# wei-zeng98/piano-a2s

Measured on AMD Instinct MI355X. Metric: training clips/sec (12 s, 5-bar), higher is better.
Workload: dtype f32

## Files before the change

include/a2s.h:

```cpp
#ifndef A2S_H
#define A2S_H
#include <stddef.h>
#include <stdint.h>
#ifdef __cplusplus
extern "C" {
#endif

#define A2S_OK 0
#define A2S_ERR_ARG (-1)
#define A2S_ERR_HIP (-2)
#define A2S_ERR_WORKSPACE (-3)

const char* a2s_last_error(void);
int a2s_version(void);
long long a2s_launch_count(void);

int a2s_gemm_f32(void* stream, int M, int N, int K, float alpha, const float* A, long sAm, long sAk,
                 const float* B, long sBk, long sBn, float beta, float* C, long ldc, const float* bias, int act,
                 int batch, long bsA, long bsB, long bsC, int splitk, float* workspace, size_t workspace_bytes);
int a2s_gemm_f32_affine(void* stream, int M, int N, int K, float alpha, const float* A, long sAm, long sAk, const float* B, long sBk,
                        long sBn, float beta, float* C, long ldc, const float* bias, int act, int batch, long bsA, long bsB, long bsC,
                        int splitk, float* workspace, size_t workspace_bytes, const float* a_scale, const float* a_shift, int a_period,
                        const float* b_scale, const float* b_shift, int b_period);
int a2s_gemm_f32_bnstats(void* stream, int M, int N, int K, const float* A, long sAm, long sAk, const float* B, long sBk, long sBn, float* C, long ldc,
                         const float* y, const float* mean, const float* invstd, const float* scale, const float* shift, int period, float* partial);
int a2s_gemm_f32_affine_scaled(void* stream, int M, int N, int K, float alpha, const float* A, long sAm, long sAk, const float* B, long sBk,
                               long sBn, float beta, float* C, long ldc, const float* bias, int act, int batch, long bsA, long bsB, long bsC,
                               int splitk, float* workspace, size_t workspace_bytes, const float* a_scale, const float* a_shift, int a_period,
                               const float* b_scale, const float* b_shift, int b_period, const float* a_absmax, const float* b_absmax);
int a2s_gemm_f32_bnstats_scaled(void* stream, int M, int N, int K, const float* A, long sAm, long sAk, const float* B, long sBk, long sBn, float* C, long ldc,
                                const float* y, const float* mean, const float* invstd, const float* scale, const float* shift, int period, float* partial,
                                const float* a_absmax, const float* b_absmax);
int a2s_linear_dgrad_bnstats(void* stream, int M, int N, int K, const float* dz, long lda, const float* Wt, float* da, long ldc, const float* y,
                             const float* mean, const float* invstd, const float* scale, const float* shift, int period, float* partial,
                             const float* dz_absmax, const float* w_absmax, float* workspace, size_t workspace_bytes, float* da_absmax_out);
int a2s_linear_fwd(void* stream, int M, int N, int K, const float* y, long lda, const float* W, float* z, long ldc, const float* scale, const float* shift,
                   int period, const float* y_absmax, const float* w_absmax, float* workspace, size_t workspace_bytes);
int a2s_linear_fwd_eligible(int M, int N, int K, int period);
int a2s_linear_wgrad(void* stream, int M, int N, int K, const float* dz, long ldz, const float* y, long lda, float* G, long ldg, const float* scale,
                     const float* shift, int period, const float* dz_absmax, const float* y_absmax, float* workspace, size_t workspace_bytes);
size_t a2s_linear_wgrad_ws_bytes(int M, int K);
int a2s_linear_wgrad_eligible(int M, int N, int K, int period);
int a2s_tallk_wgrad(void* stream, int M, int Np, int K, const float* P, long ldp, const float* A, long lda, float* G, long ldg, int transposed, float* bias,
                    const float* p_absmax, const float* a_absmax, float* workspace, size_t workspace_bytes);
size_t a2s_tallk_wgrad_ws_bytes(int M, int Np, int K);
int a2s_tallk_wgrad_eligible(int M, int Np, int K, long ldp, long lda, long ldg, int transposed);
size_t a2s_linear_dgrad_ws_bytes(int N, int K);
int a2s_linear_dgrad_blocks(int M);
int a2s_linear_dgrad_eligible(int M, int N, int K, int period);
int a2s_absmax(void* stream, const float* x, long n, float* out);
int a2s_gemm_bnstats_blocks(int M, int period);
size_t a2s_gemm_workspace_bytes(int M, int N, int batch, int splitk);
int a2s_gemm_pick_splitk(int M, int N, int K, int batch);
void a2s_gemm_debug_tile(int cfg);
int a2s_debug_set(const char* key, int value);
int a2s_debug_get(const char* key);
int a2s_env_check(void);
int a2s_persist_abort_latch(void* device_word);

int a2s_conv3x3(void* stream, const float* x, const float* w, float* y, const float* in_scale, const float* in_shift,
                float* stat_partial, int B, int T, int F, int Cin, int Cout, int flip, float* workspace);
int a2s_conv3x3_ranged(void* stream, const float* x, const float* w, float* y, const float* in_scale, const float* in_shift, const float* in_absmax,
                       float* stat_partial, float* out_absmax, int B, int T, int F, int Cin, int Cout, float* workspace);
int a2s_conv3x3_stat_blocks(int B, int T, int F, int Cin);
int a2s_conv3x3_dgrad_bnstats(void* stream, const float* dy, const float* w, float* g, const float* yl, const float* yl_mean, const float* yl_invstd,
                              const float* yl_scale, const float* yl_shift, float* stat_partial, int B, int T, int F, int Cin, int Cout,
                              float* workspace);
int a2s_bn_bwd_from_partial(void* stream, const float* g, const float* x, const float* mean, const float* invstd, const float* scale, const float* shift,
                            float* dgamma, float* dbeta, float* dx , const float* partial, int nblocks, float* c12, long rows, int C, int F);
int a2s_conv3x3_dgrad_bnstats_scaled(void* stream, const float* dy, const float* w, float* g, const float* yl, const float* yl_mean, const float* yl_invstd,
                                     const float* yl_scale, const float* yl_shift, float* stat_partial, int B, int T, int F, int Cin, int Cout,
                                     float* workspace, const float* dy_absmax);
int a2s_conv3x3_dgrad_bnstats_ranged(void* stream, const float* dy, const float* w, float* g, const float* yl, const float* yl_mean, const float* yl_invstd,
                                     const float* yl_scale, const float* yl_shift, float* stat_partial, int B, int T, int F, int Cin, int Cout,
                                     float* workspace, const float* dy_absmax, float* g_absmax_out);
int a2s_bn_bwd_from_partial_amax(void* stream, const float* g, const float* x, const float* mean, const float* invstd, const float* scale, const float* shift,
                                 float* dgamma, float* dbeta, float* dx, const float* partial, int nblocks, float* c12, long rows, int C, int F,
                                 float* dx_absmax);
size_t a2s_conv3x3_workspace_floats(int Cin);
int a2s_bn_finalize(void* stream, const float* partial, int nblocks, int C, double count, const float* gamma,
                    const float* beta, float* running_mean, float* running_var, long long* num_batches_tracked,
                    float* mean, float* invstd, float* scale, float* shift, float eps, float momentum, int training);
int a2s_bn_relu_apply(void* stream, const float* x, float* y, const float* scale, const float* shift, long n, int C, int F);
int a2s_col_stats(void* stream, const float* x, float* partial, long rows, int C, int rows_per_block);
int a2s_bn1d_relu_dropout(void* stream, const float* x, float* y, const float* scale, const float* shift,
                          const uint8_t* keep_mask, float inv_keep, long n, int C);

int a2s_gru_gates_fwd(void* stream, const float* gi, long ldgi, const float* gh, long ldgh, const float* hprev, long ldhp,
                      float* hout, long ldho, float* hout2, long ldho2, float* save, int R, int H);
int a2s_gru_seq_fwd(void* stream, const float* gi_all, long gi_bstride, long gi_tstride, const float* w_hh,
                    const float* b_hh, float* out, long out_bstride, long out_tstride, float* hbuf, float* gh,
                    float* save, float* hn, int B, int T, int H, int reverse, float* workspace, size_t workspace_bytes);

int a2s_attn_step_fwd(void* stream, const float* keys, const float* enc, const float* q, long ldq, const float* v,
                      float* ctx, long ldctx, float* ctx2, long ldctx2, float* attw, int B, int T, int H,
                      const int* n_done, int n_rows_total, float* workspace);
int a2s_attn_step_fwd_rows(void* stream, const float* keys, const float* enc, const float* q, long ldq, const float* v, float* ctx,
                           long ldctx, float* ctx2, long ldctx2, float* attw, int R, int T, int H, float* workspace, int n_clips,
                           const int* clip_order, const int* clip_rank, const int* row_until, int n_active, int step);
size_t a2s_attn_workspace_floats(int B, int T, int H);
size_t a2s_attn_workspace_floats_fused(int n_clips, int T, int H, int groups);

int a2s_log_softmax_rows(void* stream, const float* x, long ldx, float* y, long ldy, int* argmax_out, int R, int V);
int a2s_embed_rows(void* stream, const float* table, const long long* ids64, const int* ids32, long id_stride,
                   int const_id, float* out, long ldo, int col0, int R, int E, const uint8_t* keep_mask, float inv_keep);

typedef struct a2s_note_dec_args {
    const float* attn_w; const float* attn_b; const float* attn_v;
    const float* w_ih; const float* w_hh; const float* b_ih; const float* b_hh;
    const float* out_w; const float* out_b; const float* emb;
    const float* keys; const float* enc;
    float* h; float* x; float* q; float* gates; float* attw; float* o;
    float* gh; float* gi; float* logits;
    float* probs; long probs_bstride;
    const long long* gt; long gt_bstride;
    const uint8_t* tf_flags;
    const uint8_t* drop; float inv_keep;
    int* argmax_out; long am_bstride;
    int* eos_seen; long long* lengths; int* n_done;
    int* steps_exec;
    float* attn_ws;
    float* gemm_ws; size_t gemm_ws_bytes;
    int* t_base;
    const int* clip_order;
    const int* clip_rank;
    const int* row_until;
    const int* n_active;
    int n_clips;
    const int* m_active;
    const int* row_list;
    const int* n_rows_active;
    int R, T, H, E, V, steps, poll, eos_id;
    int use_graph;
    float* step_ws; size_t step_ws_floats;
    const int* tf_flags_dev;
    float* persist_ws; size_t persist_ws_bytes;
} a2s_note_dec_args;
int a2s_note_decoder_fwd(void* stream, const a2s_note_dec_args* args, int* steps_done);
int a2s_grammar_argmax_rows(void* stream, const float* x, long ldx, float* y, long ldy, const signed char* next_state, int n_states, int* row_state,
                            int* choice_out, int R, int V);
int a2s_note_decoder_fwd_grammar(void* stream, const a2s_note_dec_args* args, const signed char* next_state, int n_states, int* row_state, int* steps_done);
int a2s_grammar_launches(void);
#define A2S_BEAM_MAX 4
typedef struct a2s_beam_args {
    int K; float alpha;
    const signed char* next_state; int n_states;
    int pad_id;
    int* row_state;
    float* score; int* finished;
    int* done_count;
    int* token_hist; int* parent_hist; float* score_hist;
    float* probs_scratch;
    int* ids_out; long long* lengths_out; float* score_out;
} a2s_beam_args;
int a2s_note_decoder_fwd_beam(void* stream, const a2s_note_dec_args* args, const a2s_beam_args* beam, int* steps_done);
int a2s_beam_step(void* stream, const a2s_beam_args* beam, const float* logits, long ldl, const float* emb, float* xnext, long ldx, float* h, int h_cols,
                  float* q, int q_cols, int* n_done, int* steps_exec, int B, int V, int E, int t, int max_steps, int eos_id);
int a2s_beam_backtrack(void* stream, const a2s_beam_args* beam, float* probs, long probs_bstride, const int* steps_exec, int B, int V, int max_steps, int eos_id);
int a2s_beam_launches(void);
typedef struct a2s_align_args {
    float* attw_step;
    int* peak; float* weight; float* centroid;
    long out_stride;
    const signed char* next_state; int n_states;
    int* row_state;
} a2s_align_args;
int a2s_attn_align_rows(void* stream, const float* attw, long ldw, int R, int T, int* peak_out, float* weight_out, float* centroid_out, long out_stride);
int a2s_note_decoder_fwd_align(void* stream, const a2s_note_dec_args* args, const a2s_align_args* align, int* steps_done);
int a2s_align_launches(void);

int a2s_render_notes(void* stream, const int* programs, int rows_per_clip, int n_samples, float* wave, long wave_bstride, int B);
int a2s_render_launches(void);
int a2s_note_decoder_fwd_pair(void* stream_upper, void* stream_lower, const a2s_note_dec_args* upper, const a2s_note_dec_args* lower,
                              const int* pair_order, const int* pair_rank, const int* pair_n_active, int* steps_done_upper, int* steps_done_lower);
size_t a2s_note_step_workspace_floats(int H, int E);
size_t a2s_note_decoder_persist_ws_bytes(int n_clips, int R, int steps);
size_t a2s_note_decoder_bwd_persist_ws_bytes(int n_clips);

int a2s_staff_emb_fwd(void* stream, const float* note_emb, const float* const* gru_w, const long long* ids64,
                      const int* ids32, long id_bstride, const long long* lengths, long len_stride, float* out,
                      long ldo, int col0, float* hsave, int R, int maxlen, int E, int S);


int a2s_log_softmax_bwd_rows(void* stream, const float* g, const float* y, long outer_stride, int inner, float* dx,
                             int R, int V, int n_outer, int time_major);
int a2s_gru_gates_bwd(void* stream, const float* dh_a, long lda, const float* dh_b, long ldb, const float* save,
                      const float* hprev, long ldhp, float* dgi, long ldgi, float* dgh, long ldgh, float* dgh2, long ldgh2,
                      float* dhprev, long lddp, int R, int H);
int a2s_attn_step_bwd(void* stream, const float* keys, const float* enc, const float* q, long ldq, const float* v,
                      const float* attw, const float* ctx, long ldctx, const float* dctx_a, long ldda, const float* dctx_b,
                      long lddb, float* dctx_out, long lddo, float* dq, long lddq, float* ds_out, int B, int T, int H, float* workspace);
int a2s_attn_step_bwd_rows(void* stream, const float* keys, const float* enc, const float* q, long ldq, const float* v, const float* attw,
                           const float* ctx, long ldctx, const float* dctx_a, long ldda, const float* dctx_b, long lddb, float* dctx_out,
                           long lddo, float* dq, long lddq, float* ds_out, int R, int T, int H, float* workspace, int n_clips,
                           const int* clip_order, const int* clip_rank, const int* row_until, int n_active, int step);
int a2s_attn_dk_accum(void* stream, const float* keys, const float* q_all, const float* ds_all, const float* v, float* dK,
                      float* dv_partial, int B, int T, int S, int H, const int* row_until, int groups);
int a2s_attn_dk_blocks(int B, int T);
int a2s_attn_denc_accum(void* stream, const float* attw_all, const float* dctx_all, float* dEnc, int B, int T, int S, int H2,
// ... 95 lines not shown
```

piano_a2s_amd/csrc/a2s_api.hip:

```cpp
#define A2S_SWITCHES_IMPL
#include "a2s_internal.h"

thread_local char a2s_err_msg[512] = {0};
long long a2s_launch_counter = 0;

#define ST ((hipStream_t)stream)

extern "C" {

const char* a2s_last_error(void) { return a2s_err_msg; }
int a2s_version(void) { return 1; }
long long a2s_launch_count(void) { return __atomic_load_n(&a2s_launch_counter, __ATOMIC_RELAXED); }

int a2s_gemm_f32(void* stream, int M, int N, int K, float alpha, const float* A, long sAm, long sAk, const float* B, long sBk,
                 long sBn, float beta, float* C, long ldc, const float* bias, int act, int batch, long bsA, long bsB, long bsC,
                 int splitk, float* workspace, size_t workspace_bytes) {
    return a2s_gemm_impl(ST, M, N, K, alpha, A, sAm, sAk, B, sBk, sBn, beta, C, ldc, bias, act, batch, bsA, bsB, bsC, splitk,
                         workspace, workspace_bytes);
}
int a2s_gemm_f32_affine(void* stream, int M, int N, int K, float alpha, const float* A, long sAm, long sAk, const float* B, long sBk,
                        long sBn, float beta, float* C, long ldc, const float* bias, int act, int batch, long bsA, long bsB, long bsC,
                        int splitk, float* workspace, size_t workspace_bytes, const float* a_scale, const float* a_shift, int a_period,
                        const float* b_scale, const float* b_shift, int b_period) {
    return a2s_gemm_affine_impl(ST, M, N, K, alpha, A, sAm, sAk, B, sBk, sBn, beta, C, ldc, bias, act, batch, bsA, bsB, bsC, splitk,
                                workspace, workspace_bytes, a_scale, a_shift, a_period, b_scale, b_shift, b_period,
                                nullptr, nullptr, nullptr, nullptr, nullptr, nullptr, 0, 0, nullptr, nullptr);
}
int a2s_gemm_f32_affine_scaled(void* stream, int M, int N, int K, float alpha, const float* A, long sAm, long sAk, const float* B, long sBk,
                               long sBn, float beta, float* C, long ldc, const float* bias, int act, int batch, long bsA, long bsB, long bsC,
                               int splitk, float* workspace, size_t workspace_bytes, const float* a_scale, const float* a_shift, int a_period,
                               const float* b_scale, const float* b_shift, int b_period, const float* a_absmax, const float* b_absmax) {
    return a2s_gemm_affine_impl(ST, M, N, K, alpha, A, sAm, sAk, B, sBk, sBn, beta, C, ldc, bias, act, batch, bsA, bsB, bsC, splitk,
                                workspace, workspace_bytes, a_scale, a_shift, a_period, b_scale, b_shift, b_period,
                                nullptr, nullptr, nullptr, nullptr, nullptr, nullptr, 0, 1, a_absmax, b_absmax);
}
int a2s_gemm_f32_bnstats_scaled(void* stream, int M, int N, int K, const float* A, long sAm, long sAk, const float* B, long sBk, long sBn, float* C, long ldc,
                                const float* y, const float* mean, const float* invstd, const float* scale, const float* shift, int period, float* partial,
                                const float* a_absmax, const float* b_absmax) {
    return a2s_gemm_affine_impl(ST, M, N, K, 1.f, A, sAm, sAk, B, sBk, sBn, 0.f, C, ldc, nullptr, 0, 1, 0, 0, 0, 1, nullptr, 0,
                                nullptr, nullptr, 0, nullptr, nullptr, 0, y, mean, invstd, scale, shift, partial, period, 1, a_absmax, b_absmax);
}
int a2s_absmax(void* stream, const float* x, long n, float* out) { return a2s_absmax_impl(ST, x, n, out); }
int a2s_linear_dgrad_bnstats(void* stream, int M, int N, int K, const float* dz, long lda, const float* Wt, float* da, long ldc, const float* y,
                             const float* mean, const float* invstd, const float* scale, const float* shift, int period, float* partial,
                             const float* dz_absmax, const float* w_absmax, float* workspace, size_t workspace_bytes, float* da_absmax_out) {
    return a2s_linear_dgrad_bnstats_impl(ST, M, N, K, dz, lda, Wt, 1, K, da, ldc, y, mean, invstd, scale, shift, period, partial, dz_absmax, w_absmax,
                                         workspace, workspace_bytes, da_absmax_out);
}
size_t a2s_linear_dgrad_ws_bytes(int N, int K) { return a2s_linear_dgrad_ws_bytes_impl(N, K); }
int a2s_linear_fwd(void* stream, int M, int N, int K, const float* y, long lda, const float* W, float* z, long ldc, const float* scale, const float* shift,
                   int period, const float* y_absmax, const float* w_absmax, float* workspace, size_t workspace_bytes) {
    return a2s_linear_fwd_impl(ST, M, N, K, y, lda, W, z, ldc, scale, shift, period, y_absmax, w_absmax, workspace, workspace_bytes);
}
int a2s_linear_wgrad(void* stream, int M, int N, int K, const float* dz, long ldz, const float* y, long lda, float* G, long ldg, const float* scale,
                     const float* shift, int period, const float* dz_absmax, const float* y_absmax, float* workspace, size_t workspace_bytes) {
    return a2s_linear_wgrad_impl(ST, M, N, K, dz, ldz, y, lda, G, ldg, scale, shift, period, dz_absmax, y_absmax, workspace, workspace_bytes);
}
size_t a2s_linear_wgrad_ws_bytes(int M, int K) { return a2s_linear_wgrad_ws_bytes_impl(M, K); }
int a2s_linear_wgrad_eligible(int M, int N, int K, int period) { return a2s_linear_wgrad_ok(M, N, K, 256, 4, 4, period, nullptr, nullptr, nullptr) ? 1 : 0; }
int a2s_tallk_wgrad(void* stream, int M, int Np, int K, const float* P, long ldp, const float* A, long lda, float* G, long ldg, int transposed, float* bias,
                    const float* p_absmax, const float* a_absmax, float* workspace, size_t workspace_bytes) {
    return a2s_tallk_wgrad_impl(ST, M, Np, K, P, ldp, A, lda, G, ldg, transposed, bias, p_absmax, a_absmax, workspace, workspace_bytes);
}
size_t a2s_tallk_wgrad_ws_bytes(int M, int Np, int K) { return a2s_tallk_wgrad_ws_bytes_impl(M, Np, K); }
int a2s_tallk_wgrad_eligible(int M, int Np, int K, long ldp, long lda, long ldg, int transposed) {
    return a2s_tallk_wgrad_ok(M, Np, K, ldp, lda, ldg, transposed, nullptr, nullptr, nullptr, nullptr) ? 1 : 0;
}
int a2s_linear_fwd_eligible(int M, int N, int K, int period) { return a2s_linear_fwd_ok(M, N, K, 4, 4, period, nullptr, nullptr, nullptr) ? 1 : 0; }
int a2s_linear_dgrad_blocks(int M) { return a2s_linear_dgrad_blocks_impl(M); }
int a2s_linear_dgrad_eligible(int M, int N, int K, int period) {
    return a2s_linear_dgrad_ok(M, N, K, 4, 1, K, 4, period, nullptr, nullptr, nullptr, nullptr) ? 1 : 0;
}
int a2s_gemm_f32_bnstats(void* stream, int M, int N, int K, const float* A, long sAm, long sAk, const float* B, long sBk, long sBn, float* C, long ldc,
                         const float* y, const float* mean, const float* invstd, const float* scale, const float* shift, int period, float* partial) {
    return a2s_gemm_affine_impl(ST, M, N, K, 1.f, A, sAm, sAk, B, sBk, sBn, 0.f, C, ldc, nullptr, 0, 1, 0, 0, 0, 1, nullptr, 0,
                                nullptr, nullptr, 0, nullptr, nullptr, 0, y, mean, invstd, scale, shift, partial, period, 0, nullptr, nullptr);
}
int a2s_gemm_bnstats_blocks(int M, int period) { return a2s_cdiv(M, 128) * a2s_gemm_bnstats_slots(period); }
size_t a2s_gemm_workspace_bytes(int M, int N, int batch, int splitk) { return a2s_gemm_workspace_bytes_impl(M, N, batch, splitk); }
int a2s_gemm_pick_splitk(int M, int N, int K, int batch) { return a2s_gemm_pick_splitk_impl(M, N, K, batch); }
void a2s_gemm_debug_tile(int cfg) { a2s_gemm_debug_tile_impl(cfg); }
size_t a2s_note_step_workspace_floats(int H, int E) { return a2s_note_step_workspace_floats_impl(H, E); }
int a2s_debug_set(const char* key, int value) {
    if (!key) return A2S_ERR_ARG;
    const int id = a2s_switch_find(key);
    if (id >= 0) { a2s_switch_store(id, value); return A2S_OK; }
    if (!strcmp(key, "attn_deferred_fast")) { a2s_attn_deferred_fast = value ? 1 : 0; return A2S_OK; }
    if (!strcmp(key, "tallk_wgrad")) { a2s_tallk_wgrad_on = value ? 1 : 0; return A2S_OK; }
    if (!strcmp(key, "tallk_wgrad_max_splits")) { a2s_tallk_wgrad_max_splits = value > 0 ? value : 0; return A2S_OK; }
    if (!strcmp(key, "gemm_tile")) { a2s_gemm_debug_tile_impl(value); return A2S_OK; }
    snprintf(a2s_err_msg, sizeof(a2s_err_msg), "a2s_debug_set: unknown key %s", key);
    return A2S_ERR_ARG;
}
int a2s_env_check(void) {
    if (const char* e = a2s_switch_env_error()) A2S_FAIL(A2S_ERR_ARG, "%s: expected a decimal number >= 0", e);
    return A2S_OK;
}

int a2s_persist_abort_latch(void* device_word) { a2s_persist_latch_set(device_word); return A2S_OK; }

int a2s_debug_get(const char* key) {
    if (!key) return -1;
    const int id = a2s_switch_find(key);
    if (id == A2S_SW_attn_pair_fused_rows) return a2s_attn_pair_fused_rows();
    if (id >= 0) return a2s_sw((a2s_switch)id);
    if (!strcmp(key, "attn_pair_launches")) return (int)a2s_attn_pair_launches();
    if (!strcmp(key, "attn_pair_bwd_launches")) return (int)a2s_attn_pair_bwd_launches();
    if (!strcmp(key, "attn_deferred_fast")) return a2s_attn_deferred_fast;
    if (!strcmp(key, "tallk_wgrad")) return a2s_tallk_wgrad_on;
    if (!strcmp(key, "tallk_wgrad_max_splits")) return a2s_tallk_wgrad_max_splits;
    if (!strcmp(key, "tallk_wgrad_launches")) return (int)a2s_tallk_wgrad_launches();
    if (!strcmp(key, "attn_dk_ahead_launches")) return (int)a2s_attn_dk_ahead_launches();
    if (!strcmp(key, "attn_denc_launches")) return (int)a2s_attn_denc_launches();
    if (!strcmp(key, "dec_mid_launches")) return a2s_dec_mid_launches();
    if (!strcmp(key, "dec_persist_launches")) return a2s_dec_persist_launches();
    if (!strcmp(key, "edit_distance_launches")) return (int)a2s_edit_distance_launches();
    if (!strcmp(key, "conv_rows16_c20_launches")) return (int)a2s_conv_rows16_c20_launches();
    if (!strcmp(key, "device_cus")) return a2s_device_geometry().cus;
    if (!strcmp(key, "device_xccs")) return a2s_device_geometry().xccs;
    return -1;
}

int a2s_conv3x3(void* stream, const float* x, const float* w, float* y, const float* in_scale, const float* in_shift,
                float* stat_partial, int B, int T, int F, int Cin, int Cout, int flip, float* workspace) {
    return a2s_conv3x3_impl(ST, x, w, y, in_scale, in_shift, stat_partial, B, T, F, Cin, Cout, flip, workspace, nullptr, nullptr, nullptr, nullptr, nullptr, nullptr,
                            nullptr, nullptr);
}
int a2s_conv3x3_ranged(void* stream, const float* x, const float* w, float* y, const float* in_scale, const float* in_shift, const float* in_absmax,
                       float* stat_partial, float* out_absmax, int B, int T, int F, int Cin, int Cout, float* workspace) {
    return a2s_conv3x3_impl(ST, x, w, y, in_scale, in_shift, stat_partial, B, T, F, Cin, Cout, 0, workspace, nullptr, nullptr, nullptr, nullptr, nullptr, nullptr,
                            in_absmax, out_absmax);
}
int a2s_conv3x3_dgrad_bnstats(void* stream, const float* dy, const float* w, float* g, const float* yl, const float* yl_mean, const float* yl_invstd,
                              const float* yl_scale, const float* yl_shift, float* stat_partial, int B, int T, int F, int Cin, int Cout,
                              float* workspace) {
    if (!yl) { snprintf(a2s_err_msg, sizeof(a2s_err_msg), "conv3x3_dgrad_bnstats: yl is required"); return A2S_ERR_ARG; }
    return a2s_conv3x3_impl(ST, dy, w, g, nullptr, nullptr, stat_partial, B, T, F, Cin, Cout, 1, workspace, yl, yl_mean, yl_invstd, yl_scale, yl_shift, nullptr, nullptr, nullptr);
}
int a2s_conv3x3_dgrad_bnstats_scaled(void* stream, const float* dy, const float* w, float* g, const float* yl, const float* yl_mean, const float* yl_invstd,
                                     const float* yl_scale, const float* yl_shift, float* stat_partial, int B, int T, int F, int Cin, int Cout,
                                     float* workspace, const float* dy_absmax) {
    if (!yl) { snprintf(a2s_err_msg, sizeof(a2s_err_msg), "conv3x3_dgrad_bnstats_scaled: yl is required"); return A2S_ERR_ARG; }
    return a2s_conv3x3_impl(ST, dy, w, g, nullptr, nullptr, stat_partial, B, T, F, Cin, Cout, 1, workspace, yl, yl_mean, yl_invstd, yl_scale, yl_shift, dy_absmax, nullptr, nullptr);
}
int a2s_conv3x3_dgrad_bnstats_ranged(void* stream, const float* dy, const float* w, float* g, const float* yl, const float* yl_mean, const float* yl_invstd,
                                     const float* yl_scale, const float* yl_shift, float* stat_partial, int B, int T, int F, int Cin, int Cout,
                                     float* workspace, const float* dy_absmax, float* g_absmax_out) {
    if (!yl) { snprintf(a2s_err_msg, sizeof(a2s_err_msg), "conv3x3_dgrad_bnstats_ranged: yl is required"); return A2S_ERR_ARG; }
    return a2s_conv3x3_impl(ST, dy, w, g, nullptr, nullptr, stat_partial, B, T, F, Cin, Cout, 1, workspace, yl, yl_mean, yl_invstd, yl_scale, yl_shift, dy_absmax, nullptr, g_absmax_out);
}
int a2s_bn_bwd_from_partial(void* stream, const float* g, const float* x, const float* mean, const float* invstd, const float* scale, const float* shift,
                            float* dgamma, float* dbeta, float* dx, const float* partial, int nblocks, float* c12, long rows, int C, int F) {
    return a2s_bn_bwd_from_partial_impl(ST, g, x, mean, invstd, scale, shift, dgamma, dbeta, dx, partial, nblocks, c12, rows, C, F, nullptr);
}
int a2s_bn_bwd_from_partial_amax(void* stream, const float* g, const float* x, const float* mean, const float* invstd, const float* scale, const float* shift,
                                 float* dgamma, float* dbeta, float* dx, const float* partial, int nblocks, float* c12, long rows, int C, int F,
                                 float* dx_absmax) {
    return a2s_bn_bwd_from_partial_impl(ST, g, x, mean, invstd, scale, shift, dgamma, dbeta, dx, partial, nblocks, c12, rows, C, F, dx_absmax);
}
size_t a2s_conv3x3_workspace_floats(int Cin) { return a2s_conv3x3_workspace_floats_impl(Cin); }
int a2s_conv3x3_stat_blocks(int B, int T, int F, int Cin) { return a2s_conv3x3_stat_blocks_impl(B, T, F, Cin); }
int a2s_bn_finalize(void* stream, const float* partial, int nblocks, int C, double count, const float* gamma, const float* beta,
                    float* running_mean, float* running_var, long long* nbt, float* mean, float* invstd, float* scale,
                    float* shift, float eps, float momentum, int training) {
    return a2s_bn_finalize_impl(ST, partial, nblocks, C, count, gamma, beta, running_mean, running_var, nbt, mean, invstd, scale,
                                shift, eps, momentum, training);
}
int a2s_bn_relu_apply(void* stream, const float* x, float* y, const float* scale, const float* shift, long n, int C, int F) {
    return a2s_bn_relu_apply_impl(ST, x, y, scale, shift, n, C, F);
}
int a2s_col_stats(void* stream, const float* x, float* partial, long rows, int C, int rows_per_block) {
    return a2s_col_stats_impl(ST, x, partial, rows, C, rows_per_block);
}
int a2s_bn1d_relu_dropout(void* stream, const float* x, float* y, const float* scale, const float* shift, const uint8_t* keep_mask,
                          float inv_keep, long n, int C) {
    return a2s_bn1d_relu_dropout_impl(ST, x, y, scale, shift, keep_mask, inv_keep, n, C);
}
int a2s_gru_gates_fwd(void* stream, const float* gi, long ldgi, const float* gh, long ldgh, const float* hprev, long ldhp,
                      float* hout, long ldho, float* hout2, long ldho2, float* save, int R, int H) {
    return a2s_gru_gates_fwd_impl(ST, gi, ldgi, gh, ldgh, hprev, ldhp, hout, ldho, hout2, ldho2, save, R, H);
}
int a2s_gru_seq_fwd(void* stream, const float* gi_all, long gi_bstride, long gi_tstride, const float* w_hh, const float* b_hh,
                    float* out, long out_bstride, long out_tstride, float* hbuf, float* gh, float* save, float* hn, int B, int T,
                    int H, int reverse, float* workspace, size_t workspace_bytes) {
    return a2s_gru_seq_fwd_impl(ST, gi_all, gi_bstride, gi_tstride, w_hh, b_hh, out, out_bstride, out_tstride, hbuf, gh, save, hn,
                                B, T, H, reverse, workspace, workspace_bytes);
}
int a2s_attn_step_fwd(void* stream, const float* keys, const float* enc, const float* q, long ldq, const float* v, float* ctx,
                      long ldctx, float* ctx2, long ldctx2, float* attw, int B, int T, int H, const int* n_done, int n_rows_total, float* workspace) {
    return a2s_attn_step_fwd_impl(ST, keys, enc, q, ldq, v, ctx, ldctx, ctx2, ldctx2, attw, B, T, H, n_done, n_rows_total, workspace, nullptr);
}
int a2s_attn_step_fwd_rows(void* stream, const float* keys, const float* enc, const float* q, long ldq, const float* v, float* ctx,
                           long ldctx, float* ctx2, long ldctx2, float* attw, int R, int T, int H, float* workspace, int n_clips,
                           const int* clip_order, const int* clip_rank, const int* row_until, int n_active, int step) {
    a2s_attn_rows rows = {clip_order, clip_rank, row_until, n_clips, n_active, step};
    return a2s_attn_step_fwd_impl(ST, keys, enc, q, ldq, v, ctx, ldctx, ctx2, ldctx2, attw, R, T, H, nullptr, 0, workspace, &rows);
}
size_t a2s_attn_workspace_floats(int B, int T, int H) { return a2s_attn_workspace_floats_impl(B, T, H, 1); }
size_t a2s_attn_workspace_floats_fused(int n_clips, int T, int H, int groups) { return a2s_attn_workspace_floats_impl(n_clips, T, H, groups); }
int a2s_log_softmax_rows(void* stream, const float* x, long ldx, float* y, long ldy, int* argmax_out, int R, int V) {
    return a2s_log_softmax_rows_impl(ST, x, ldx, y, ldy, argmax_out, R, V);
}
int a2s_embed_rows(void* stream, const float* table, const long long* ids64, const int* ids32, long id_stride, int const_id,
                   float* out, long ldo, int col0, int R, int E, const uint8_t* keep_mask, float inv_keep) {
    return a2s_embed_rows_impl(ST, table, ids64, ids32, id_stride, const_id, out, ldo, col0, R, E, keep_mask, inv_keep);
}
int a2s_note_decoder_fwd(void* stream, const a2s_note_dec_args* args, int* steps_done) {
    if (!args) { snprintf(a2s_err_msg, sizeof(a2s_err_msg), "note_decoder_fwd: null args"); return A2S_ERR_ARG; }
    return a2s_note_decoder_fwd_impl(ST, *args, steps_done);
}
int a2s_grammar_argmax_rows(void* stream, const float* x, long ldx, float* y, long ldy, const signed char* next_state, int n_states, int* row_state,
                            int* choice_out, int R, int V) {
    return a2s_grammar_argmax_rows_impl(ST, x, ldx, y, ldy, next_state, n_states, row_state, choice_out, R, V);
}
int a2s_note_decoder_fwd_grammar(void* stream, const a2s_note_dec_args* args, const signed char* next_state, int n_states, int* row_state, int* steps_done) {
    if (!args) { snprintf(a2s_err_msg, sizeof(a2s_err_msg), "note_decoder_fwd_grammar: null args"); return A2S_ERR_ARG; }
    const a2s_grammar_ref g = {next_state, n_states, row_state};
    return a2s_note_decoder_fwd_grammar_impl(ST, *args, g, steps_done);
}
int a2s_grammar_launches(void) { return a2s_grammar_launches_impl(); }
int a2s_note_decoder_fwd_beam(void* stream, const a2s_note_dec_args* args, const a2s_beam_args* beam, int* steps_done) {
    if (!args || !beam) { snprintf(a2s_err_msg, sizeof(a2s_err_msg), "note_decoder_fwd_beam: null args"); return A2S_ERR_ARG; }
    return a2s_note_decoder_fwd_beam_impl(ST, *args, *beam, steps_done);
}
int a2s_beam_step(void* stream, const a2s_beam_args* beam, const float* logits, long ldl, const float* emb, float* xnext, long ldx, float* h, int h_cols,
                  float* q, int q_cols, int* n_done, int* steps_exec, int B, int V, int E, int t, int max_steps, int eos_id) {
    if (!beam) { snprintf(a2s_err_msg, sizeof(a2s_err_msg), "beam_step: null args"); return A2S_ERR_ARG; }
    const a2s_beam_args& g = *beam;
    const BeamStepArgs a = {logits, ldl, emb, xnext, ldx, h, h_cols, q, q_cols, g.next_state, g.n_states, g.row_state, g.score, g.finished, g.done_count,
                            g.token_hist, g.parent_hist, g.score_hist, g.probs_scratch, n_done, steps_exec, B, g.K, V, E, t, max_steps, eos_id, g.pad_id};
    return a2s_beam_step_finalize_impl(ST, a);
}
int a2s_beam_backtrack(void* stream, const a2s_beam_args* beam, float* probs, long probs_bstride, const int* steps_exec, int B, int V, int max_steps, int eos_id) {
    if (!beam) { snprintf(a2s_err_msg, sizeof(a2s_err_msg), "beam_backtrack: null args"); return A2S_ERR_ARG; }
    const a2s_beam_args& g = *beam;
    const BeamBackArgs a = {g.score, g.token_hist, g.parent_hist, g.probs_scratch, probs, probs_bstride, g.ids_out, (long)max_steps, g.lengths_out, g.score_out,
                            steps_exec, g.alpha, B, g.K, V, max_steps, eos_id, g.pad_id};
    return a2s_beam_backtrack_impl(ST, a);
}
int a2s_beam_launches(void) { return a2s_beam_launches_impl(); }
int a2s_attn_align_rows(void* stream, const float* attw, long ldw, int R, int T, int* peak_out, float* weight_out, float* centroid_out, long out_stride) {
    return a2s_attn_align_rows_impl(ST, attw, ldw, R, T, peak_out, weight_out, centroid_out, out_stride);
}
int a2s_note_decoder_fwd_align(void* stream, const a2s_note_dec_args* args, const a2s_align_args* align, int* steps_done) {
    if (!args || !align) { snprintf(a2s_err_msg, sizeof(a2s_err_msg), "note_decoder_fwd_align: null args"); return A2S_ERR_ARG; }
    return a2s_note_decoder_fwd_align_impl(ST, *args, *align, steps_done);
}
int a2s_align_launches(void) { return a2s_align_launches_impl(); }
int a2s_render_notes(void* stream, const int* programs, int rows_per_clip, int n_samples, float* wave, long wave_bstride, int B) {
    return a2s_render_notes_impl(ST, programs, rows_per_clip, n_samples, wave, wave_bstride, B);
}
int a2s_render_launches(void) { return a2s_render_launches_impl(); }
int a2s_note_decoder_fwd_pair(void* stream_upper, void* stream_lower, const a2s_note_dec_args* upper, const a2s_note_dec_args* lower,
                              const int* pair_order, const int* pair_rank, const int* pair_n_active, int* steps_done_upper, int* steps_done_lower) {
    if (!upper || !lower) { snprintf(a2s_err_msg, sizeof(a2s_err_msg), "note_decoder_fwd_pair: null args"); return A2S_ERR_ARG; }
    return a2s_note_decoder_fwd_pair_impl((hipStream_t)stream_upper, (hipStream_t)stream_lower, *upper, *lower, pair_order, pair_rank, pair_n_active,
                                          steps_done_upper, steps_done_lower);
}
int a2s_staff_emb_fwd(void* stream, const float* note_emb, const float* const* gru_w, const long long* ids64, const int* ids32,
                      long id_bstride, const long long* lengths, long len_stride, float* out, long ldo, int col0, float* hsave,
                      int R, int maxlen, int E, int S) {
    if (!gru_w) { snprintf(a2s_err_msg, sizeof(a2s_err_msg), "staff_emb_fwd: null weight table"); return A2S_ERR_ARG; }
    return a2s_staff_emb_fwd_impl(ST, note_emb, gru_w, ids64, ids32, id_bstride, lengths, len_stride, out, ldo, col0, hsave, R,
                                  maxlen, E, S);
// ... 163 lines not shown
```

piano_a2s_amd/csrc/a2s_internal.h:

```cpp
#pragma once
#include "a2s_common.h"
#include "../../include/a2s.h"
#include "a2s_switches.h"

static inline int a2s_attn_pair_fused_rows(void) {
    const int cap = a2s_sw(A2S_SW_dec_fused_max_rows), v = a2s_sw(A2S_SW_attn_pair_fused_rows);
    return v < cap ? v : cap;
}
static inline unsigned a2s_persist_dbg(void) {
    return (a2s_sw(A2S_SW_persist_force_agent) ? PERSIST_DBG_FORCE_AGENT : 0u) | (a2s_sw(A2S_SW_persist_inject_abort) ? PERSIST_DBG_INJECT_ABORT : 0u);
}

int a2s_absmax_impl(hipStream_t st, const float* x, long n, float* out);
size_t a2s_gemm_workspace_bytes_impl(int M, int N, int batch, int splitk);
int a2s_gemm_pick_splitk_impl(int M, int N, int K, int batch);
int a2s_gemm_bnstats_slots(int period);
void a2s_gemm_debug_tile_impl(int cfg);
int a2s_gemm_affine_impl(hipStream_t st, int M, int N, int K, float alpha, const float* A, long sAm, long sAk,
    const float* B, long sBk, long sBn, float beta, float* C, long ldc, const float* bias, int act,
    int batch, long bsA, long bsB, long bsC, int splitk, float* ws, size_t ws_bytes,
    const float* a_scale, const float* a_shift, int a_period, const float* b_scale, const float* b_shift, int b_period,
    const float* ep_y, const float* ep_mean, const float* ep_invstd, const float* ep_scale, const float* ep_shift,
    float* ep_partial, int ep_period, int two_term, const float* a_absmax, const float* b_absmax);
int a2s_gemm_impl(hipStream_t st, int M, int N, int K, float alpha, const float* A, long sAm, long sAk,
    const float* B, long sBk, long sBn, float beta, float* C, long ldc, const float* bias, int act,
    int batch, long bsA, long bsB, long bsC, int splitk, float* ws, size_t ws_bytes);

size_t a2s_linear_dgrad_ws_bytes_impl(int N, int K);
int a2s_linear_dgrad_blocks_impl(int M);
bool a2s_linear_dgrad_ok(int M, int N, int K, long lda, long sBk, long sBn, long ldc, int period, const void* A, const void* B, const void* C, const void* y);
int a2s_linear_dgrad_bnstats_impl(hipStream_t st, int M, int N, int K, const float* A, long lda, const float* Wt, long sBk, long sBn, float* C, long ldc,
    const float* ep_y, const float* mean, const float* invstd, const float* scale, const float* shift, int period,
    float* partial, const float* a_absmax, const float* b_absmax, float* ws, size_t ws_bytes, float* c_absmax_out);
bool a2s_linear_fwd_ok(int M, int N, int K, long lda, long ldc, int period, const void* A, const void* W, const void* C);
int a2s_linear_fwd_impl(hipStream_t st, int M, int N, int K, const float* A, long lda, const float* W, float* C, long ldc, const float* a_scale,
    const float* a_shift, int period, const float* a_absmax, const float* w_absmax, float* ws, size_t ws_bytes);
size_t a2s_linear_wgrad_ws_bytes_impl(int M, int K);
bool a2s_linear_wgrad_ok(int M, int N, int K, long ldz, long lda, long ldg, int period, const void* dz, const void* A, const void* G);
int a2s_linear_wgrad_impl(hipStream_t st, int M, int N, int K, const float* dz, long ldz, const float* A, long lda, float* G, long ldg, const float* a_scale,
    const float* a_shift, int period, const float* dz_absmax, const float* a_absmax, float* ws, size_t ws_bytes);
extern int a2s_tallk_wgrad_on;
extern int a2s_tallk_wgrad_max_splits;
long a2s_tallk_wgrad_launches(void);
size_t a2s_tallk_wgrad_ws_bytes_impl(int M, int Np, int K);
bool a2s_tallk_wgrad_ok(int M, int Np, int K, long ldp, long lda, long ldg, int transposed, const void* P, const void* A, const void* G, const void* bias);
int a2s_tallk_wgrad_impl(hipStream_t st, int M, int Np, int K, const float* P, long ldp, const float* A, long lda, float* G, long ldg, int transposed,
    float* bias, const float* p_absmax, const float* a_absmax, float* ws, size_t ws_bytes);

int a2s_act_bound_impl(hipStream_t st, const float* scale, const float* shift, const float* absmax, int C, float* out);
size_t a2s_conv3x3_workspace_floats_impl(int Cin);
int a2s_conv3x3_impl(hipStream_t st, const float* x, const float* w, float* y, const float* in_scale,
    const float* in_shift, float* stat_partial, int B, int T, int F, int Cin, int Cout, int flip, float* ws,
    const float* yl, const float* yl_mean, const float* yl_invstd, const float* yl_scale, const float* yl_shift,
    const float* x_absmax, const float* in_absmax, float* out_absmax);
int a2s_conv3x3_stat_blocks_impl(int B, int T, int F, int Cin);
int a2s_bn_finalize_impl(hipStream_t st, const float* partial, int nblocks, int C, double count, const float* gamma,
    const float* beta, float* running_mean, float* running_var, long long* nbt, float* mean,
    float* invstd, float* scale, float* shift, float eps, float momentum, int training);
int a2s_bn_relu_apply_impl(hipStream_t st, const float* x, float* y, const float* scale, const float* shift, long n, int C, int F);
int a2s_col_stats_impl(hipStream_t st, const float* x, float* partial, long rows, int C, int rows_per_block);
int a2s_bn1d_relu_dropout_impl(hipStream_t st, const float* x, float* y, const float* scale, const float* shift,
    const uint8_t* mask, float inv_keep, long n, int C);
size_t a2s_conv3x3_wgrad_workspace_bytes_impl(int Cin, int Cout);
int a2s_conv3x3_wgrad_impl(hipStream_t st, const float* dy, const float* x, const float* in_scale, const float* in_shift, float* dW,
    float* ws, size_t ws_bytes, int B, int T, int F, int Cin, int Cout, const float* bn_y, const float* bn_mean,
    const float* bn_invstd, const float* bn_scale, const float* bn_shift, const float* bn_c12, float* dy_out,
    const float* dy_absmax, const float* act_absmax);
int a2s_bn_bwd_impl(hipStream_t st, const float* g, const float* x, const float* mean, const float* invstd, const float* scale,
    const float* shift, const uint8_t* mask, float inv_keep, float* dgamma, float* dbeta, float* dx, float* partial,
    float* c12, long rows, int C, int F, float* dx_absmax);
int a2s_bn_bwd_from_partial_impl(hipStream_t st, const float* g, const float* x, const float* mean, const float* invstd, const float* scale,
    const float* shift, float* dgamma, float* dbeta, float* dx, const float* partial, int nblocks, float* c12,
    long rows, int C, int F, float* dx_absmax);
int a2s_bn_bwd_stats_impl(hipStream_t st, const float* g, const float* x, const float* mean, const float* invstd, const float* scale,
    const float* shift, const uint8_t* mask, float inv_keep, float* partial, float* sums, long rows, int C, int F);
int a2s_bn_bwd_apply_impl(hipStream_t st, const float* g, const float* x, const float* mean, const float* invstd, const float* scale,
    const float* shift, const uint8_t* mask, float inv_keep, const float* sums_local, const float* sums_global,
    double count_global, float* dgamma, float* dbeta, float* dx, float* c12, long rows, int C, int F);
int a2s_bn_bwd_sums_from_partial_impl(hipStream_t st, const float* partial, int nblocks, int C, float* sums);
int a2s_bn_bwd_c12_from_sums_impl(hipStream_t st, const float* sums_local, const float* sums_global, double count_global, float* dgamma, float* dbeta,
    float* c12, int C);
size_t a2s_bn_bwd_partial_floats_impl(long rows, int C, int F);

int a2s_channel_absmax_impl(hipStream_t st, const float* x, long rows, int C, int F, float* out);
bool a2s_conv_rows_eligible(int F, int Cin);
int a2s_conv_rows_blocks(int B, int T, int F);
size_t a2s_conv_rows_workspace_floats(int Cin);
long a2s_conv_rows16_c20_launches(void);
int a2s_conv3x3_rows_impl(hipStream_t st, const float* x, const float* w, float* y, const float* in_scale, const float* in_shift,
    const float* in_absmax, float* stat_partial, float* out_absmax, int B, int T, int F, int Cin, int Cout, int flip,
    float* ws, const float* yl, const float* yl_mean, const float* yl_invstd, const float* yl_scale, const float* yl_shift,
    const float* x_absmax);

bool a2s_wgrad_rows_eligible(int F, int Cin, int Cout);
int a2s_conv3x3_wgrad_rows_bn_impl(hipStream_t st, const float* g, const float* y, const float* mean, const float* invstd, const float* scale,
    const float* shift, const float* c12, const float* g_absmax, int g_absmax_n, const float* y_absmax, float* dz_out,
    float* dz_absmax_out, const float* x, const float* in_scale, const float* in_shift, float* dW, float* ws, size_t ws_bytes,
    int B, int T, int F, int Cin, int Cout, const float* act_absmax);
int a2s_conv3x3_wgrad_rows_impl(hipStream_t st, const float* dy, const float* x, const float* in_scale, const float* in_shift, float* dW, float* ws,
    size_t ws_bytes, int B, int T, int F, int Cin, int Cout, const float* dy_absmax, const float* act_absmax);

struct StepFinArgs {
    const float* logits; long ldl;
    float* probs; long probs_bstride;
    const long long* gt; long gt_bstride;
    const float* emb;
    float* xnext; long ldx;
    const uint8_t* drop; float inv_keep;
    int* argmax_out; long am_bstride;
    int* eos_seen; long long* lengths; int* n_done; int* steps_exec;
    const int* t_base;
    const int* row_until;
    int n_clips;
    int R, V, E, t, teacher_force, eos_id, max_t;
};
struct a2s_grammar_ref { const signed char* next; int n_states; int* row_state; };
int a2s_gru_gates_fwd_impl(hipStream_t st, const float* gi, long ldgi, const float* gh, long ldgh, const float* hprev,
    long ldhp, float* hout, long ldho, float* hout2, long ldho2, float* save, int R, int H);
int a2s_gru_bptt_step_impl(hipStream_t st, const float* dgh, const float* w_hh_t, const float* dhz_in, const float* dout, long ld_dout,
    const float* save, const float* hprev, long ld_hprev, float* dgi, long ld_dgi, float* dgh_out, float* dgh2,
    long ld_dgh2, float* dhz_out, int R, int H);
int a2s_skinny_gemm_acc_impl(hipStream_t st, const float* A, long lda, const float* Bt, long ldb, float* Cm, long ldc, int R, int N, int K);
int a2s_gru_seq_fwd_impl(hipStream_t st, const float* gi_all, long gi_bstride, long gi_tstride, const float* w_hh,
    const float* b_hh, float* out, long out_bstride, long out_tstride, float* hbuf, float* gh,
    float* save, float* hn, int B, int T, int H, int reverse, float* ws, size_t ws_bytes);
int a2s_attn_step_fwd_impl(hipStream_t st, const float* Kmat, const float* enc, const float* q, long ldq, const float* v,
    float* ctx, long ldctx, float* ctx2, long ldctx2, float* attw, int B, int T, int H,
    const int* n_done, int n_rows_total, float* ws, const a2s_attn_rows* rows = nullptr, a2s_attn_deferred* defer = nullptr);
int a2s_log_softmax_rows_impl(hipStream_t st, const float* x, long ldx, float* y, long ldy, int* argmax_out, int R, int V);
int a2s_embed_rows_impl(hipStream_t st, const float* table, const long long* ids64, const int* ids32, long id_stride,
    int const_id, float* out, long ldo, int col0, int R, int E, const uint8_t* drop, float inv_keep);
int a2s_note_decoder_fwd_impl(hipStream_t st, const a2s_note_dec_args& a, int* steps_done);
int a2s_note_decoder_fwd_grammar_impl(hipStream_t st, const a2s_note_dec_args& a, const a2s_grammar_ref& g, int* steps_done);
int a2s_note_decoder_fwd_pair_impl(hipStream_t su, hipStream_t sl, const a2s_note_dec_args& au, const a2s_note_dec_args& al, const int* pair_order,
    const int* pair_rank, const int* pair_n_active, int* done_u, int* done_l);
int a2s_staff_emb_fwd_impl(hipStream_t st, const float* note_emb, const float* const* w ,
    const long long* ids64, const int* ids32, long id_bstride, const long long* lengths,
    long len_stride, float* out, long ldo, int col0, float* hsave, int R, int maxlen, int E, int S);
size_t a2s_attn_workspace_floats_impl(int B, int T, int H, int groups);
size_t a2s_attn_bulk_lds(size_t shm, int n_active, int backward);
long a2s_attn_pair_launches(void);

int a2s_log_softmax_bwd_rows_impl(hipStream_t st, const float* g, const float* y, long outer_stride, int inner, float* dx,
    int R, int V, int n_outer, int time_major);
int a2s_gru_gates_bwd_impl(hipStream_t st, const float* dh_a, long lda, const float* dh_b, long ldb, const float* save,
    const float* hprev, long ldhp, float* dgi, long ldgi, float* dgh, long ldgh, float* dgh2, long ldgh2,
    float* dhprev, long lddp, int R, int H);
int a2s_attn_step_bwd_impl(hipStream_t st, const float* Kmat, const float* enc, const float* q, long ldq, const float* v,
    const float* attw, const float* ctx, long ldctx, const float* dctx_a, long ldda, const float* dctx_b,
    long lddb, float* dctx_out, long lddo, float* dq, long lddq, float* ds_out, int B, int T, int H, float* ws,
    const a2s_attn_rows* rows = nullptr);
int a2s_attn_dk_accum_impl(hipStream_t st, const float* Kmat, const float* q_all, const float* ds_all, const float* v,
    float* dK, float* dv_partial, int B, int T, int S, int H, const int* row_until, int groups);
int a2s_attn_denc_accum_impl(hipStream_t st, const float* attw_all, const float* dctx_all, float* dEnc, int B, int T, int S, int H2,
    const int* row_until, int groups);
long a2s_attn_dk_ahead_launches(void);
long a2s_attn_denc_launches(void);
int a2s_col_sum_impl(hipStream_t st, const float* x, long ld, float* out, long rows, int C, float alpha, float beta, float* ws, size_t ws_floats);
int a2s_embed_scatter_add_impl(hipStream_t st, float* table_grad, const long long* ids64, const int* ids32, long id_stride,
    int const_id, const float* g, long ldg, int col0, int R, int E, const uint8_t* drop, float inv_keep);
int a2s_ew_act_bwd_impl(hipStream_t st, const float* g, const float* y, float* dx, long n, int act);
int a2s_note_decoder_bwd_impl(hipStream_t st, const a2s_note_dec_bwd_args& a);
int a2s_note_decoder_bwd_pair_impl(hipStream_t su, hipStream_t sl, const a2s_note_dec_bwd_args& au, const a2s_note_dec_bwd_args& al, const int* pair_order,
    const int* pair_rank, const int* pair_n_active);
int a2s_gru_seq_bwd_impl(hipStream_t st, const float* dout, long do_bstride, long do_tstride, const float* out, long out_bstride,
    long out_tstride, const float* gates, const float* w_hh, const float* dhn, float* dgi_all, float* dgh_shift,
    float* dgh_first, float* dhbuf, float* dgh_tmp, int B, int T, int H, int reverse, float* ws, size_t ws_bytes,
    float* ranges_out, int* ranges_valid);
int a2s_staff_emb_bwd_impl(hipStream_t st, const float* note_emb, const float* const* w, float* const* grads_dev, float* note_emb_grad,
    const long long* ids64, const int* ids32, long id_bstride, const long long* lengths, long len_stride,
    const float* dout, long lddo, int col0, const float* hsave, int R, int maxlen, int E, int S);
long a2s_attn_pair_bwd_launches(void);

size_t a2s_note_step_fused_head_floats(void);
size_t a2s_note_step_workspace_floats_impl(int H, int E);
int a2s_dec_mid_launches(void);
bool a2s_dec_step_fusable(int R, int H, int E, int V, const void* const* ptrs, int nptrs, const float* ws, size_t ws_floats, bool greedy = false);
int a2s_note_step_fused_fwd(hipStream_t st, const a2s_note_dec_args& a, int si, int so, int sv, int sv_next, int t, const int* t_base, int tf, bool last,
    int nrows, const int* rowmap, const a2s_attn_deferred* defer = nullptr);
int a2s_note_step_fused_bwd_prepare(hipStream_t st, const a2s_note_dec_bwd_args& a);
int a2s_note_step_fused_bwd(hipStream_t st, const a2s_note_dec_bwd_args& a, int s, const float* dh_in, float* dh_out, const a2s_attn_rows* rows,
    int nrows, const int* rowmap);
bool a2s_note_step_mid_ok(int H, int E, const void* const* ptrs, int nptrs);
int a2s_note_step_mid_gru(hipStream_t st, const a2s_note_dec_args& a, int si, int so, int sv, int sv_next, int nrows, const int* rowmap);
bool a2s_note_step_mid_bwd_ok(const a2s_note_dec_bwd_args& a);
int a2s_note_step_mid_bwd(hipStream_t st, const a2s_note_dec_bwd_args& a, int s, float* dh_out, int nrows, const int* rowmap);
int a2s_note_step_mid_bwd_query(hipStream_t st, const a2s_note_dec_bwd_args& a, int s, float* dh_out, int nrows, const int* rowmap);

bool a2s_grammar_ref_ok(const a2s_grammar_ref& g, int R, int V);
int a2s_grammar_argmax_rows_impl(hipStream_t st, const float* x, long ldx, float* y, long ldy, const signed char* next, int n_states, int* row_state,
    int* choice_out, int R, int V);
int a2s_grammar_step_finalize_impl(hipStream_t st, const StepFinArgs& a, const a2s_grammar_ref& g);
int a2s_grammar_launches_impl(void);
// ... 69 lines not shown
```

piano_a2s_amd/csrc/a2s_linear.hip:

```cpp
#include "a2s_internal.h"

#define LIN_BM 128
#define LIN_K 256
#define LIN_RS 288
#define LIN_NTH 512
#define LIN_LDS (2 * 2 * LIN_BM * LIN_RS)

typedef unsigned lu32x4 __attribute__((ext_vector_type(4)));

struct LinDgradArgs {
    const float* A; long lda;
    const unsigned char* planes;
    float* C; long ldc;
    const float* ep_y;
    const float* mean; const float* invstd; const float* scale; const float* shift;
    float* partial;
    const float* a_absmax; const float* b_absmax;
    int M, N, period, channels;
    float* c_absmax_out;
};

__global__ __launch_bounds__(256) void lin_pack_planes_k(const float* __restrict__ W, long ld, int N, int K, const float* __restrict__ absmax,
                                                         unsigned char* __restrict__ out) {
    const long id = (long)blockIdx.x * 256 + threadIdx.x;
    const int kgroups = K >> 3, nks = K >> 5;
    const int n = (int)(id / kgroups), kg = (int)(id % kgroups);
    if (n >= N) return;
    const float ps = ldexpf(1.f, pow2_scale_exp(*absmax, 12));
    const f32x4 v0 = *reinterpret_cast<const f32x4*>(W + (long)n * ld + kg * 8);
    const f32x4 v1 = *reinterpret_cast<const f32x4*>(W + (long)n * ld + kg * 8 + 4);
    float x[8];
#pragma unroll
    for (int i = 0; i < 4; ++i) { x[i] = __builtin_amdgcn_fmed3f(v0[i] * ps, -65000.f, 65000.f); x[4 + i] = __builtin_amdgcn_fmed3f(v1[i] * ps, -65000.f, 65000.f); }
    lu32x4 hi, lo;
#pragma unroll
    for (int i = 0; i < 4; ++i) { unsigned h, l; split2_pair_f16(x[2 * i], x[2 * i + 1], h, l); hi[i] = h; lo[i] = l; }
    const int nt = n >> 4, lr = n & 15, ks = kg >> 2, lk = kg & 3;
    unsigned char* o = out + ((((long)nt * nks + ks) * 2) * 64 + (lk * 16 + lr)) * 16;
    *reinterpret_cast<lu32x4*>(o) = hi;
    *reinterpret_cast<lu32x4*>(o + 64 * 16) = lo;
}

__global__ __launch_bounds__(LIN_NTH) void lin_dgrad_bnstats(LinDgradArgs a) {
    __shared__ __attribute__((aligned(16))) unsigned char lds[LIN_LDS];
    const int tid = threadIdx.x, lane = tid & 63, wave = tid >> 6, lr = lane & 15, lk = lane >> 4;
    const int m0 = blockIdx.x * LIN_BM;
    const int ka = pow2_scale_exp(*a.a_absmax, 12), kb = pow2_scale_exp(*a.b_absmax, 12);
    const float psa = ldexpf(1.f, ka), unscale = ldexpf(1.f, -(ka + kb));

    {
        f32x4 v[16];
#pragma unroll
        for (int i = 0; i < 16; ++i) {
            const int slot = tid + LIN_NTH * i, row = slot >> 6, k = (slot & 63) * 4;
            v[i] = (f32x4){0.f, 0.f, 0.f, 0.f};
            if (m0 + row < a.M) v[i] = *reinterpret_cast<const f32x4*>(a.A + (long)(m0 + row) * a.lda + k);
        }
#pragma unroll
        for (int i = 0; i < 16; ++i) {
            const int slot = tid + LIN_NTH * i, row = slot >> 6, k = (slot & 63) * 4;
            float x[4];
#pragma unroll
            for (int j = 0; j < 4; ++j) x[j] = __builtin_amdgcn_fmed3f(v[i][j] * psa, -65000.f, 65000.f);
            uint2 hi, lo;
            split2_pair_f16(x[0], x[1], hi.x, lo.x);
            split2_pair_f16(x[2], x[3], hi.y, lo.y);
            const int blk = k >> 7, off = (k & 127) * 2;
            *reinterpret_cast<uint2*>(lds + ((blk * 2 + 0) * LIN_BM + row) * LIN_RS + off) = hi;
            *reinterpret_cast<uint2*>(lds + ((blk * 2 + 1) * LIN_BM + row) * LIN_RS + off) = lo;
        }
    }
    __syncthreads();

    const int ntiles = (a.N + 255) >> 8;
    const unsigned lane_off = (unsigned)(lr * a.ldc + lk * 4) * 4u;
    float s1 = 0.f, s2 = 0.f, vmax = 0.f;
    int cur_c = -1;
    auto flush = [&]() {
        if (cur_c < 0) return;
        const float w1 = wave_sum(s1), w2 = wave_sum(s2);
        if (lane == 0) {
            float* p = a.partial + (((long)blockIdx.x * 8 + wave) * a.channels + cur_c) * 2;
            p[0] = w1; p[1] = w2;
        }
    };
    lu32x4 bf[3][2][2];
    auto load_b = [&](int n0, int ks, lu32x4 (&dst)[2][2]) {
        const unsigned char* bp = a.planes + (long)(n0 >> 4) * 8 * 2 * 64 * 16;
#pragma unroll
        for (int nt = 0; nt < 2; ++nt)
#pragma unroll
            for (int sp = 0; sp < 2; ++sp) dst[nt][sp] = *reinterpret_cast<const lu32x4*>(bp + ((long)(nt * 8 + ks) * 2 + sp) * 1024 + (unsigned)lane * 16u);
    };
    if (wave * 32 < a.N) { load_b(wave * 32, 0, bf[0]); load_b(wave * 32, 1, bf[1]); }
    for (int j = 0; j < ntiles; ++j) {
        const int n0 = j * 256 + wave * 32;
        if (n0 >= a.N) break;
        f32x4 yq[8][2];
        auto load_y = [&](int mt) {
            const int m = m0 + mt * 16 + lr;
#pragma unroll
            for (int nt = 0; nt < 2; ++nt) {
#if defined(LIN_X) && LIN_X >= 1 && LIN_X != 4
                yq[mt][nt] = (f32x4){1.f, 1.f, 1.f, 1.f};
#else
                yq[mt][nt] = (f32x4){0.f, 0.f, 0.f, 0.f};
                if (m < a.M)
                    yq[mt][nt] = *reinterpret_cast<const f32x4*>(reinterpret_cast<const char*>(a.ep_y + (long)(m0 + mt * 16) * a.ldc + n0 + nt * 16) + lane_off);
#endif
            }
        };
#pragma unroll
        for (int mt = 0; mt < 3; ++mt) load_y(mt);
        f32x4 acc[8][2];
#pragma unroll
        for (int mt = 0; mt < 8; ++mt)
#pragma unroll
            for (int nt = 0; nt < 2; ++nt) acc[mt][nt] = (f32x4){0.f, 0.f, 0.f, 0.f};
#pragma unroll
        for (int ks = 0; ks < 8; ++ks) {
#if defined(LIN_X) && LIN_X >= 3
            if (ks + 2 < 8 && a.M < 0) load_b(n0, ks + 2, bf[(ks + 2) % 3]);
#else
            if (ks + 2 < 8) load_b(n0, ks + 2, bf[(ks + 2) % 3]);
#endif
#pragma unroll
            for (int half = 0; half < 2; ++half) {
                lu32x4 af[2][4];
#pragma unroll
                for (int sp = 0; sp < 2; ++sp)
#pragma unroll
                    for (int q = 0; q < 4; ++q)
                        af[sp][q] = *reinterpret_cast<const lu32x4*>(lds + (((ks >> 2) * 2 + sp) * LIN_BM + (half * 4 + q) * 16 + lr) * LIN_RS + (ks & 3) * 64 + lk * 16);
#define LIN_PRODUCT(SA, SB)                                                                                                   \
                _Pragma("unroll") for (int nt = 0; nt < 2; ++nt)                                                              \
                    _Pragma("unroll") for (int q = 0; q < 4; ++q)                                                             \
                        acc[half * 4 + q][nt] = __builtin_amdgcn_mfma_f32_16x16x32_f16(__builtin_bit_cast(f16x8, bf[ks % 3][nt][SB]), \
                                                                                       __builtin_bit_cast(f16x8, af[SA][q]), acc[half * 4 + q][nt], 0, 0, 0);
                LIN_PRODUCT(1, 0) LIN_PRODUCT(0, 1) LIN_PRODUCT(0, 0)
#undef LIN_PRODUCT
            }
        }
        if (n0 + 256 < a.N) { load_b(n0 + 256, 0, bf[0]); load_b(n0 + 256, 1, bf[1]); }
#pragma unroll
        for (int mt = 3; mt < 8; ++mt) load_y(mt);
        const int c = n0 / a.period;
        if (c != cur_c) { flush(); s1 = 0.f; s2 = 0.f; cur_c = c; }
        const float mean = a.mean[c], invstd = a.invstd[c], sc = a.scale[c], sh = a.shift[c];
#pragma unroll
        for (int mt = 0; mt < 8; ++mt) {
            const int m = m0 + mt * 16 + lr;
            if (m >= a.M) continue;
#pragma unroll
            for (int nt = 0; nt < 2; ++nt) {
                f32x4 v = acc[mt][nt];
#pragma unroll
                for (int r = 0; r < 4; ++r) { v[r] *= unscale; vmax = fmaxf(vmax, fabsf(v[r])); }
#if defined(LIN_X) && LIN_X >= 2
                if (v[0] == 123.456f)
#endif
                *reinterpret_cast<f32x4*>(reinterpret_cast<char*>(a.C + (long)(m0 + mt * 16) * a.ldc + n0 + nt * 16) + lane_off) = v;
#pragma unroll
                for (int r = 0; r < 4; ++r) {
                    const float gm = (fmaf(yq[mt][nt][r], sc, sh) > 0.f) ? v[r] : 0.f;
                    s1 += gm; s2 = fmaf(gm * (yq[mt][nt][r] - mean), invstd, s2);
                }
            }
        }
    }
    flush();
    if (a.c_absmax_out) {
        const float m = wave_max(vmax);
        if (lane == 0 && m > 0.f) atomicMax(reinterpret_cast<unsigned*>(a.c_absmax_out), __float_as_uint(m));
    }
}

size_t a2s_linear_dgrad_ws_bytes_impl(int N, int K) { return (K > 0 && K % 32 == 0 && N > 0) ? (size_t)N * K * 2 * 2 : 0; }
int a2s_linear_dgrad_blocks_impl(int M) { return M > 0 ? ((M + LIN_BM - 1) / LIN_BM) * 8 : 0; }

bool a2s_linear_dgrad_ok(int M, int N, int K, long lda, long sBk, long sBn, long ldc, int period, const void* A, const void* B, const void* C, const void* y) {
    return K == LIN_K && M >= LIN_BM && N >= 256 && N % 32 == 0 && period > 0 && period % 32 == 0 && N % period == 0 && N / period <= 4096 && sBk == 1 && sBn == K &&
           lda % 4 == 0 && ldc % 4 == 0 && (((uintptr_t)A | (uintptr_t)B | (uintptr_t)C | (uintptr_t)y) % 16 == 0);
}

int a2s_linear_dgrad_bnstats_impl(hipStream_t st, int M, int N, int K, const float* A, long lda, const float* Wt, long sBk, long sBn, float* C, long ldc,
                                  const float* ep_y, const float* mean, const float* invstd, const float* scale, const float* shift, int period,
                                  float* partial, const float* a_absmax, const float* b_absmax, float* ws, size_t ws_bytes, float* c_absmax_out) {
    A2S_REQUIRE(A && Wt && C && ep_y && mean && invstd && scale && shift && partial && a_absmax && b_absmax && ws, "linear_dgrad_bnstats: null argument");
    A2S_REQUIRE(a2s_linear_dgrad_ok(M, N, K, lda, sBk, sBn, ldc, period, A, Wt, C, ep_y),
                "linear_dgrad_bnstats: needs K = 256, M >= 128, N >= 256, N %% 32 == 0, period %% 32 == 0, a k-contiguous weight (N x K) and 16-byte aligned rows");
    A2S_REQUIRE(((uintptr_t)ws % 16 == 0) && ws_bytes >= a2s_linear_dgrad_ws_bytes_impl(N, K), "linear_dgrad_bnstats: workspace too small (%zu bytes needed)",
                a2s_linear_dgrad_ws_bytes_impl(N, K));
    const int channels = N / period, nblk = a2s_linear_dgrad_blocks_impl(M);
    hipError_t e = hipMemsetAsync(partial, 0, sizeof(float) * 2 * (size_t)nblk * channels, st);
    if (e != hipSuccess) A2S_FAIL(A2S_ERR_HIP, "linear_dgrad_bnstats memset: %s", hipGetErrorString(e));
    unsigned char* planes = reinterpret_cast<unsigned char*>(ws);
    hipLaunchKernelGGL(lin_pack_planes_k, dim3((unsigned)(((long)N * (K / 8) + 255) / 256)), dim3(256), 0, st, Wt, (long)K, N, K, b_absmax, planes);
    A2S_CHECK_LAUNCH("lin_pack_planes_k");
    LinDgradArgs a{A, lda, planes, C, ldc, ep_y, mean, invstd, scale, shift, partial, a_absmax, b_absmax, M, N, period, channels, c_absmax_out};
    hipLaunchKernelGGL(lin_dgrad_bnstats, dim3((M + LIN_BM - 1) / LIN_BM), dim3(LIN_NTH), 0, st, a);
    A2S_CHECK_LAUNCH("lin_dgrad_bnstats");
    return A2S_OK;
}

#define LF_RS 160
#define LF_STAGE (2 * LIN_BM * LF_RS)
#define LF_NS 3

struct LinFwdArgs {
    const float* A; long lda;
    const unsigned char* planes;
    float* C; long ldc;
    const float* a_scale; const float* a_shift;
    const float* a_absmax; const float* b_absmax;
    int M, K, period;
};

__global__ __launch_bounds__(LIN_NTH) void lin_fwd_roles(LinFwdArgs a) {
    __shared__ __attribute__((aligned(16))) unsigned char lds[LF_NS * LF_STAGE];
    const int tid = threadIdx.x, lane = tid & 63, lr = lane & 15, lk = lane >> 4;
    const int wave = __builtin_amdgcn_readfirstlane(tid >> 6);
    const int m0 = blockIdx.x * LIN_BM;
    const int ka = a.a_absmax ? pow2_scale_exp(*a.a_absmax, 12) : 0, kb = pow2_scale_exp(*a.b_absmax, 12);
    const float psa = ldexpf(1.f, ka), unscale = ldexpf(1.f, -(ka + kb));
    const int nks = a.K >> 5, nblk = a.K >> 6, kpc = a.period >> 5;
    const bool affine = a.a_scale != nullptr;
    if (wave >= 4) {
        const int st_ = tid - 256;
        const int sk = (st_ & 15) * 4;
        const bool second = sk >= 32;
        f32x4 ar[2][8];
        auto issue_a = [&](int blk, f32x4 (&r)[8]) {
#pragma unroll
            for (int i = 0; i < 8; ++i) {
                const int row = (st_ + 256 * i) >> 4;
                r[i] = (f32x4){0.f, 0.f, 0.f, 0.f};
                if (m0 + row < a.M && blk < nblk) r[i] = __builtin_nontemporal_load(reinterpret_cast<const f32x4*>(a.A + (long)(m0 + row) * a.lda + (long)blk * 64 + sk));
            }
        };
        auto commit_a = [&](int blk, const f32x4 (&r)[8]) {
            if (blk >= nblk) return;
            const int c0 = (2 * blk) / kpc, c1 = (2 * blk + 1) / kpc;
            const float sc = affine ? (second ? a.a_scale[c1] : a.a_scale[c0]) * psa : psa, sh = affine ? (second ? a.a_shift[c1] : a.a_shift[c0]) * psa : 0.f;
            const float floor_ = affine ? 0.f : -INFINITY;
            unsigned char* st = lds + (blk % LF_NS) * LF_STAGE;
#pragma unroll
            for (int i = 0; i < 8; ++i) {
                const int row = (st_ + 256 * i) >> 4;
                float x[4];
#pragma unroll
                for (int j = 0; j < 4; ++j) x[j] = __builtin_amdgcn_fmed3f(fmaxf(fmaf(r[i][j], sc, sh), floor_), -65000.f, 65000.f);
                uint2 hi, lo;
                split2_pair_f16(x[0], x[1], hi.x, lo.x);
                split2_pair_f16(x[2], x[3], hi.y, lo.y);
                *reinterpret_cast<uint2*>(st + (0 * LIN_BM + row) * LF_RS + sk * 2) = hi;
                *reinterpret_cast<uint2*>(st + (1 * LIN_BM + row) * LF_RS + sk * 2) = lo;
            }
        };
        issue_a(0, ar[0]);
        commit_a(0, ar[0]);
        issue_a(1, ar[1]); issue_a(2, ar[0]);
#pragma unroll 1
        for (int b0 = 0; b0 < nblk; b0 += 2) {
            __syncthreads();
            commit_a(b0 + 1, ar[1]); issue_a(b0 + 3, ar[1]);
            if (b0 + 1 < nblk) {
                __syncthreads();
                commit_a(b0 + 2, ar[0]); issue_a(b0 + 4, ar[0]);
            }
        }
        return;
    }
    lu32x4 bf[2][4][2];
    auto load_b = [&](int ks, lu32x4 (&dst)[4][2]) {
        if (ks >= nks) return;
#pragma unroll
        for (int nt = 0; nt < 4; ++nt)
#pragma unroll
            for (int sp = 0; sp < 2; ++sp)
                dst[nt][sp] = *reinterpret_cast<const lu32x4*>(a.planes + (((long)(wave * 4 + nt) * nks + ks) * 2 + sp) * 1024 + (unsigned)lane * 16u);
    };
    f32x4 acc[8][4];
#pragma unroll
    for (int mt = 0; mt < 8; ++mt)
#pragma unroll
        for (int nt = 0; nt < 4; ++nt) acc[mt][nt] = (f32x4){0.f, 0.f, 0.f, 0.f};
    load_b(0, bf[0]);
    auto load_af = [&](const unsigned char* st, int h, int qt, lu32x4 (&af)[2][2]) {
#pragma unroll
        for (int sp = 0; sp < 2; ++sp)
#pragma unroll
            for (int q = 0; q < 2; ++q) af[sp][q] = *reinterpret_cast<const lu32x4*>(st + (sp * LIN_BM + (qt * 2 + q) * 16 + lr) * LF_RS + h * 64 + lk * 16);
    };
    auto multiply = [&](int qt, const lu32x4 (&af)[2][2], const lu32x4 (&b)[4][2]) {
#define LR_PRODUCT(SA, SB)                                                                                                        \
        _Pragma("unroll") for (int nt = 0; nt < 4; ++nt)                                                                          \
            _Pragma("unroll") for (int q = 0; q < 2; ++q)                                                                         \
                acc[qt * 2 + q][nt] = __builtin_amdgcn_mfma_f32_16x16x32_f16(__builtin_bit_cast(f16x8, b[nt][SB]),                \
                                                                             __builtin_bit_cast(f16x8, af[SA][q]), acc[qt * 2 + q][nt], 0, 0, 0);
        LR_PRODUCT(1, 0) LR_PRODUCT(0, 1) LR_PRODUCT(0, 0)
#undef LR_PRODUCT
    };
#pragma unroll 1
    for (int blk = 0; blk < nblk; ++blk) {
        __syncthreads();
        const unsigned char* st = lds + (blk % LF_NS) * LF_STAGE;
        lu32x4 fa[2][2], fb[2][2];
        load_af(st, 0, 0, fa);
        load_b(2 * blk + 1, bf[1]);
        __builtin_amdgcn_sched_barrier(0);
        load_af(st, 0, 1, fb); multiply(0, fa, bf[0]);
        __builtin_amdgcn_sched_barrier(0);
        load_af(st, 0, 2, fa); multiply(1, fb, bf[0]);
        __builtin_amdgcn_sched_barrier(0);
        load_af(st, 0, 3, fb); multiply(2, fa, bf[0]);
        __builtin_amdgcn_sched_barrier(0);
        load_af(st, 1, 0, fa); multiply(3, fb, bf[0]);
        __builtin_amdgcn_sched_barrier(0);
        load_b(2 * blk + 2, bf[0]);
        load_af(st, 1, 1, fb); multiply(0, fa, bf[1]);
        __builtin_amdgcn_sched_barrier(0);
        load_af(st, 1, 2, fa); multiply(1, fb, bf[1]);
        __builtin_amdgcn_sched_barrier(0);
        load_af(st, 1, 3, fb); multiply(2, fa, bf[1]);
        __builtin_amdgcn_sched_barrier(0);
        multiply(3, fb, bf[1]);
        __builtin_amdgcn_sched_barrier(0);
    }
#pragma unroll
    for (int mt = 0; mt < 8; ++mt) {
        const int m = m0 + mt * 16 + lr;
        if (m >= a.M) continue;
#pragma unroll
        for (int nt = 0; nt < 4; ++nt) {
            f32x4 v = acc[mt][nt];
#pragma unroll
            for (int r = 0; r < 4; ++r) v[r] *= unscale;
            *reinterpret_cast<f32x4*>(a.C + (long)m * a.ldc + wave * 64 + nt * 16 + lk * 4) = v;
        }
    }
}

bool a2s_linear_fwd_ok(int M, int N, int K, long lda, long ldc, int period, const void* A, const void* W, const void* C) {
    return N == 256 && M >= 1 && K >= 128 && K % 64 == 0 && (period == 0 || (period % 32 == 0 && K % period == 0)) && lda % 4 == 0 && ldc % 4 == 0 &&
           (((uintptr_t)A | (uintptr_t)W | (uintptr_t)C) % 16 == 0);
}

int a2s_linear_fwd_impl(hipStream_t st, int M, int N, int K, const float* A, long lda, const float* W, float* C, long ldc, const float* a_scale,
                        const float* a_shift, int period, const float* a_absmax, const float* w_absmax, float* ws, size_t ws_bytes) {
    A2S_REQUIRE(A && W && C && w_absmax && ws && ((a_scale == nullptr) == (a_shift == nullptr)), "linear_fwd: null argument");
    A2S_REQUIRE(a2s_linear_fwd_ok(M, N, K, lda, ldc, a_scale ? period : 0, A, W, C),
                "linear_fwd: needs N = 256, K %% 64 == 0, period %% 32 == 0 and 16-byte aligned rows");
    A2S_REQUIRE(((uintptr_t)ws % 16 == 0) && ws_bytes >= (size_t)N * K * 4, "linear_fwd: workspace too small (%zu bytes needed)", (size_t)N * K * 4);
    unsigned char* planes = reinterpret_cast<unsigned char*>(ws);
    hipLaunchKernelGGL(lin_pack_planes_k, dim3((unsigned)(((long)N * (K / 8) + 255) / 256)), dim3(256), 0, st, W, (long)K, N, K, w_absmax, planes);
    A2S_CHECK_LAUNCH("lin_pack_planes_k");
    LinFwdArgs a{A, lda, planes, C, ldc, a_scale, a_shift, a_absmax, w_absmax, M, K, a_scale ? period : K};
    hipLaunchKernelGGL(lin_fwd_roles, dim3((M + LIN_BM - 1) / LIN_BM), dim3(LIN_NTH), 0, st, a);
    A2S_CHECK_LAUNCH("lin_fwd");
    return A2S_OK;
}

struct LinWgradArgs {
    const float* A; long lda;
    const unsigned char* planes;
    float* partial;
    const float* a_scale; const float* a_shift;
    const float* a_absmax; const float* d_absmax;
    int M, K, period, nblk, blk_per_split;
    long plane_stride; int np;
    float* bias_partial;
};

__global__ __launch_bounds__(256) void lin_pack_dz_planes(const float* __restrict__ dz, long ld, int M, int nsteps, const float* __restrict__ absmax,
                                                          unsigned char* __restrict__ out) {
    const long id = (long)blockIdx.x * 256 + threadIdx.x;
    const int n = (int)(id & 255), lk = (int)((id >> 8) & 3), s = (int)(id >> 10);
    if (s >= nsteps) return;
    dz += blockIdx.y * 256;
    out += (size_t)blockIdx.y * nsteps * (16 * 2 * 1024);
    float ps = ldexpf(1.f, pow2_scale_exp(*absmax, 12));
    if ((s >> 3) & 1) ps = -ps;
    float x[8];
#pragma unroll
    for (int j = 0; j < 8; ++j) {
        const int m = s * 32 + lk * 8 + j;
        x[j] = m < M ? __builtin_amdgcn_fmed3f(dz[(long)m * ld + n] * ps, -65000.f, 65000.f) : 0.f;
    }
    lu32x4 hi, lo;
#pragma unroll
    for (int i = 0; i < 4; ++i) { unsigned h, l; split2_pair_f16(x[2 * i], x[2 * i + 1], h, l); hi[i] = h; lo[i] = l; }
    unsigned char* o = out + ((((long)s * 16 + (n >> 4)) * 2) * 64 + (lk * 16 + (n & 15))) * 16;
    *reinterpret_cast<lu32x4*>(o) = hi;
    *reinterpret_cast<lu32x4*>(o + 64 * 16) = lo;
}

template <bool BIAS>
__global__ __launch_bounds__(LIN_NTH) void lin_wgrad_roles(LinWgradArgs a) {
    __shared__ __attribute__((aligned(16))) unsigned char lds[LF_NS * LF_STAGE];
    const int tid = threadIdx.x, lane = tid & 63, lr = lane & 15, lk = lane >> 4;
    const int wave = __builtin_amdgcn_readfirstlane(tid >> 6);
    const int k0 = blockIdx.x * LIN_BM;
    const int b_lo = blockIdx.y * a.blk_per_split, b_hi = min(a.nblk, b_lo + a.blk_per_split);
    const int ka = a.a_absmax ? pow2_scale_exp(*a.a_absmax, 12) : 0, kd = pow2_scale_exp(*a.d_absmax, 12);
    const float psa = ldexpf(1.f, ka), unscale = ldexpf(1.f, -(ka + kd));
    const bool affine = a.a_scale != nullptr;
    if (wave >= 4) {
        const int st_ = tid - 256;
        const int rq = st_ & 15, cq0 = st_ >> 4;
        float sc[2], sh[2];
#pragma unroll
        for (int u = 0; u < 2; ++u) {
            const int ch = affine ? (k0 + 4 * (cq0 + 16 * u)) / a.period : 0;
            sc[u] = affine ? a.a_scale[ch] * psa : psa; sh[u] = affine ? a.a_shift[ch] * psa : 0.f;
        }
        const float floor_ = affine ? 0.f : -INFINITY;
        f32x4 ar[2][8];
        f32x4 bs[2] = {(f32x4){0.f, 0.f, 0.f, 0.f}, (f32x4){0.f, 0.f, 0.f, 0.f}};
        auto issue_a = [&](int blk, f32x4 (&r)[8]) {
#pragma unroll
            for (int u = 0; u < 2; ++u)
#pragma unroll
                for (int j = 0; j < 4; ++j) {
                    const int m = blk * 64 + 4 * rq + j;
                    r[4 * u + j] = (f32x4){0.f, 0.f, 0.f, 0.f};
                    if (m < a.M && blk < b_hi) r[4 * u + j] = __builtin_nontemporal_load(reinterpret_cast<const f32x4*>(a.A + (long)m * a.lda + k0 + 4 * (cq0 + 16 * u)));
                }
        };
        auto commit_a = [&](int blk, const f32x4 (&r)[8]) {
            if (blk >= b_hi) return;
            unsigned char* st = lds + (blk % LF_NS) * LF_STAGE;
            if (BIAS) {
#pragma unroll
                for (int u = 0; u < 2; ++u)
#pragma unroll
                    for (int j = 0; j < 4; ++j)
#pragma unroll
                        for (int c = 0; c < 4; ++c) bs[u][c] += r[4 * u + j][c];
            }
#pragma unroll
            for (int u = 0; u < 2; ++u)
#pragma unroll
                for (int c = 0; c < 4; ++c) {
                    float x[4];
#pragma unroll
                    for (int j = 0; j < 4; ++j) x[j] = __builtin_amdgcn_fmed3f(fmaxf(fmaf(r[4 * u + j][c], sc[u], sh[u]), floor_), -65000.f, 65000.f);
                    uint2 hi, lo;
                    split2_pair_f16(x[0], x[1], hi.x, lo.x);
                    split2_pair_f16(x[2], x[3], hi.y, lo.y);
                    *reinterpret_cast<uint2*>(st + (0 * LIN_BM + 4 * (cq0 + 16 * u) + c) * LF_RS + rq * 8) = hi;
                    *reinterpret_cast<uint2*>(st + (1 * LIN_BM + 4 * (cq0 + 16 * u) + c) * LF_RS + rq * 8) = lo;
                }
        };
        if (b_lo < b_hi) {
            issue_a(b_lo, ar[0]);
            commit_a(b_lo, ar[0]);
            issue_a(b_lo + 1, ar[1]); issue_a(b_lo + 2, ar[0]);
        }
#pragma unroll 1
        for (int b = b_lo; b < b_hi; b += 2) {
            __syncthreads();
            commit_a(b + 1, ar[1]); issue_a(b + 3, ar[1]);
            if (b + 1 < b_hi) {
                __syncthreads();
                commit_a(b + 2, ar[0]); issue_a(b + 4, ar[0]);
            }
        }
        if (BIAS && blockIdx.z == 0) {
#pragma unroll
            for (int u = 0; u < 2; ++u) {
#pragma unroll
                for (int c = 0; c < 4; ++c)
#pragma unroll
                    for (int o = 1; o < 16; o <<= 1) bs[u][c] += __shfl_xor(bs[u][c], o, 64);
                if (rq == 0) *reinterpret_cast<f32x4*>(a.bias_partial + (long)blockIdx.y * a.K + k0 + 4 * (cq0 + 16 * u)) = bs[u];
            }
        }
        return;
    }
    lu32x4 df[2][4][2];
    const unsigned char* planes = a.planes + blockIdx.z * a.plane_stride;
    auto load_d = [&](int step, lu32x4 (&dst)[4][2]) {
        if (step >= 2 * b_hi) return;
#pragma unroll
        for (int nt = 0; nt < 4; ++nt)
#pragma unroll
            for (int sp = 0; sp < 2; ++sp)
                dst[nt][sp] = *reinterpret_cast<const lu32x4*>(planes + ((((long)step) * 16 + wave * 4 + nt) * 2 + sp) * 1024 + (unsigned)lane * 16u);
    };
    f32x4 acc[8][4];
#pragma unroll
    for (int kt = 0; kt < 8; ++kt)
#pragma unroll
        for (int nt = 0; nt < 4; ++nt) acc[kt][nt] = (f32x4){0.f, 0.f, 0.f, 0.f};
    bool neg = false;
    auto flip = [&]() {
#pragma unroll
        for (int kt = 0; kt < 8; ++kt)
#pragma unroll
            for (int nt = 0; nt < 4; ++nt)
#pragma unroll
                for (int r = 0; r < 4; ++r) acc[kt][nt][r] = -acc[kt][nt][r];
    };
    auto load_bf = [&](const unsigned char* st, int h, int qt, lu32x4 (&f)[2][2]) {
#pragma unroll
        for (int sp = 0; sp < 2; ++sp)
#pragma unroll
            for (int q = 0; q < 2; ++q) f[sp][q] = *reinterpret_cast<const lu32x4*>(st + (sp * LIN_BM + (qt * 2 + q) * 16 + lr) * LF_RS + h * 64 + lk * 16);
    };
    auto multiply = [&](int qt, const lu32x4 (&f)[2][2], const lu32x4 (&d)[4][2]) {
#define LW_PRODUCT(SX, SD)                                                                                                        \
        _Pragma("unroll") for (int nt = 0; nt < 4; ++nt)                                                                          \
// ... 174 lines not shown
```

piano_a2s_amd/engine.py:

```python
import ctypes as C
import random as _py_random
import threading

import torch

from . import hip
from .spec import EOS, PAD, SOS, VOCAB_SIZE


def plan_note_steps(gt_rows, max_steps):
    B = gt_rows.shape[0]
    is_eos = gt_rows == EOS
    first = torch.where(is_eos.any(1), is_eos.float().argmax(1), torch.full((B,), max_steps))
    steps = int(first.max()) + 1 if bool((first < max_steps).all()) else max_steps
    steps = min(steps, max_steps)
    idx = torch.arange(1, steps + 1, dtype=torch.long)
    last = (is_eos[:, :steps].long() * idx).amax(dim=1)
    lengths = torch.where(last > 0, last, torch.full((B,), max_steps, dtype=torch.long))
    return steps, lengths


import os as _os

_GREEDY_GRAPH = _os.environ.get("A2S_GREEDY_GRAPH") == "1"
# ... 166 lines not shown
        cur = torch.cuda.current_stream()
        return (cur, cur)
    return side_streams(device)


_ISSUE_POOL = None


def fork_on_streams(device, streams, fns):
    global _ISSUE_POOL
    fork = torch.cuda.Event()
    fork.record()
    dev_index = _dev_index(device)
    caller_stream = torch.cuda.current_stream()

    def task(st, fn):
        torch.cuda.set_device(dev_index)
        if st == caller_stream:
            with torch.cuda.stream(st):
                return fn(), None
        st.wait_event(fork)
        with torch.cuda.stream(st):
            r = fn()
        done = torch.cuda.Event()
        done.record(st)
        return r, done

    if _ISSUE_POOL is None:
        from concurrent.futures import ThreadPoolExecutor
        _ISSUE_POOL = ThreadPoolExecutor(max_workers=6, thread_name_prefix="a2s-issue")
    futures = [_ISSUE_POOL.submit(task, st, fn) for st, fn in zip(streams, fns)]

    def join(wait=True):
        res = [f.result() for f in futures]
        events = [done for _, done in res if done is not None]
        if not wait:
            return [r for r, _ in res], events
        for done in events:
            torch.cuda.current_stream().wait_event(done)
        return [r for r, _ in res]
    return join


def _dist_world():
    import torch.distributed as dist
    return dist.get_world_size() if dist.is_available() and dist.is_initialized() else 0


class Engine:
    def __init__(self, cfg, sync_bn=False):
        self.cfg = cfg
        self.attn_clip_steps = []
        self.attn_shared_clip_steps = []
        self.poll = 16
        self.kern_grammar = None
        self.decoded = None
        self.beam_size = 1
        self.beam_length_penalty = 0.0
        self.beam_scores = None
        self.alignment = False
        self.alignment_out = None
        self.sync_bn = bool(sync_bn) and _dist_world() >= 1

    def _global_stats(self, partial, nblocks, C_, count):
        import torch.distributed as dist
        sums = torch.empty(2 * C_, dtype=torch.float32, device=partial.device)
        hip.check(hip.lib().a2s_col_sum(hip.stream(), hip._p(partial), 2 * C_, hip._p(sums), nblocks, 2 * C_, 1.0, 0.0, None, 0), "a2s_col_sum (bn stats)")
        dist.all_reduce(sums)
        return sums, float(count) * dist.get_world_size()

    @staticmethod
    def check_counts(count, dev):
        import torch.distributed as dist
        t = torch.tensor([float(count), -float(count)], dtype=torch.float64, device=dev)
        dist.all_reduce(t, op=dist.ReduceOp.MAX)
        hi, lo = float(t[0]), -float(t[1])
        if hi != lo:
            raise RuntimeError(f"synchronised BatchNorm: the ranks hold different numbers of frames in this step ({lo:.0f} .. {hi:.0f}); "
                               "give every rank the same batch shape (DistributedSampler pads; drop or pad an uneven last batch)")

    @staticmethod
    def _empty(*shape, dev, dtype=torch.float32):
        return torch.empty(shape, dtype=dtype, device=dev)

    def _bn(self, S, name, partial, nblocks, C_, count, training):
        dev = S[name + ".weight"].device
        mean, invstd, scale, shift = (self._empty(C_, dev=dev) for _ in range(4))
        L = hip.lib()
        self.bn_counts = getattr(self, "bn_counts", {})
        if training and self.sync_bn:
            partial, count = self._global_stats(partial, nblocks, C_, count)
            nblocks = 1
        self.bn_counts[name] = count
        hip.check(L.a2s_bn_finalize(hip.stream(), hip._p(partial), nblocks, C_, count, hip._p(S[name + ".weight"]), hip._p(S[name + ".bias"]),
                                    hip._p(S[name + ".running_mean"]), hip._p(S[name + ".running_var"]), hip._p(S[name + ".num_batches_tracked"]), hip._p(mean),
                                    hip._p(invstd), hip._p(scale), hip._p(shift), 1e-5, 0.1, 1 if training else 0), "a2s_bn_finalize")
        return mean, invstd, scale, shift

    def convstack(self, S, spec_in, training, drop_mask=None):
        L = hip.lib()
        B, _, T, F = spec_in.shape
        dev = spec_in.device
        x = spec_in.contiguous()
        chans = [(1, 20), (20, 20), (20, 40), (40, 40)]
        scale = shift = None
        saved = {"x0": x, "y": [], "bn": [], "yabs": []}
        yabs = None
        for i, (ci, co) in enumerate(chans, start=1):
            y = self._empty(B, T, co, F, dev=dev)
            nblk = L.a2s_conv3x3_stat_blocks(B, T, F, ci)
            partial = self._empty(nblk, co, 2, dev=dev) if training else None
            cws = hip.conv_workspace(ci, dev)
            yabs_out = self._empty(co, dev=dev)
            hip.conv3x3_forward(x.view(B, T, ci, F), S[f"convstack.conv{i}.weight"], y, scale, shift, partial, cws, yabs, yabs_out)
            mean, invstd, scale, shift = self._bn(S, f"convstack.bn{i}", partial, nblk, co, float(B) * T * F, training)
            saved["y"].append(y)
            saved["bn"].append((mean, invstd, scale, shift))
            saved["yabs"].append(yabs_out)
            saved.setdefault("abound", []).append(hip.act_bound(scale, shift, yabs_out))
            x, yabs = y, yabs_out
        y4 = x.view(B * T, 40 * F)
        Cf = self.cfg["conv_feature_size"]
        a4 = None
        saved["w_out_amax"] = hip.absmax(S["convstack.out.weight"])
        z = hip.linear_forward(y4, S["convstack.out.weight"], (scale, shift, F), saved["abound"][3], saved["w_out_amax"])
        rows = B * T
        rpb = 64
        nblk = (rows + rpb - 1) // rpb
        partial = None
        if training:
            partial = self._empty(nblk, Cf, 2, dev=dev)
            hip.check(L.a2s_col_stats(hip.stream(), hip._p(z), hip._p(partial), rows, Cf, rpb), "a2s_col_stats")
        mean, invstd, scale, shift = self._bn(S, "convstack.out_bn", partial, nblk, Cf, float(rows), training)
        out = self._empty(rows, Cf, dev=dev)
        hip.check(L.a2s_bn1d_relu_dropout(hip.stream(), hip._p(z), hip._p(out), hip._p(scale), hip._p(shift), hip._p(drop_mask), 1.0 / 0.8, out.numel(), Cf),
                  "a2s_bn1d_relu_dropout")
        saved.update(a4=a4, z=z, out_bn=(mean, invstd, scale, shift), drop=drop_mask)
        return out.view(B, T, Cf), saved

    def encoder(self, S, x, training):
        L = hip.lib()
        B, T, _ = x.shape
        H = self.cfg["hidden_size"]
        dev = x.device
        saved = {"layers": []}
        gws = [hip.gemm_workspace(B, dev), hip.gemm_workspace(B, dev)]
        streams = encoder_streams(dev, B)
        inp = x.reshape(B * T, -1)
        finals = []
        for layer in (0, 1):
            out = self._empty(B, T, 2 * H, dev=dev)
            lsave = {"in": inp, "dirs": []}
            in_amax = (hip.absmax(inp) if layer == 0 else hip.one(dev)) if _ENC_TWO_TERM else None
            gis = [hip.linear(inp, S[f"encoder.gru.weight_ih_{sfx}"], S[f"encoder.gru.bias_ih_{sfx}"],
                              two_term=(in_amax, hip.absmax(S[f"encoder.gru.weight_ih_{sfx}"])) if _ENC_TWO_TERM else None)
                   for sfx in (f"l{layer}", f"l{layer}_reverse")]
            def direction(d, sfx, gi):
                hbuf = self._empty(2, B, H, dev=dev)
                gh = self._empty(B, 3 * H, dev=dev)
                hn = self._empty(B, H, dev=dev)
                gates = self._empty(T, B, 4 * H, dev=dev) if training else None
                hip.check(L.a2s_gru_seq_fwd(hip.stream(), hip._p(gi), T * 3 * H, 3 * H, hip._p(S[f"encoder.gru.weight_hh_{sfx}"]),
                                            hip._p(S[f"encoder.gru.bias_hh_{sfx}"]), C.c_void_p(out.data_ptr() + 4 * d * H), T * 2 * H, 2 * H, hip._p(hbuf), hip._p(gh),
                                            hip._p(gates), hip._p(hn), B, T, H, d, hip._p(gws[d]), gws[d].numel() * 4), "a2s_gru_seq_fwd")
                return {"gi": gi, "gates": gates, "hn": hn, "scratch": (hbuf, gh)}

            join = fork_on_streams(dev, streams, [lambda d=d, sfx=sfx: direction(d, sfx, gis[d])
                                                  for d, sfx in enumerate((f"l{layer}", f"l{layer}_reverse"))])
            for rec in join():
                finals.append(rec["hn"])
                lsave["dirs"].append(rec)
            lsave["out"] = out
            saved["layers"].append(lsave)
            inp = out.view(B * T, 2 * H)
        W, bias = S["encoder.fc.weight"], S["encoder.fc.bias"]
        hidden = self._empty(B, 2 * H, dev=dev)
        for l in (0, 1):
            hf, hr = finals[2 * l], finals[2 * l + 1]
            hip.gemm(hf, H, 1, W, 1, 2 * H, hidden, 2 * H, B, H, H, bias=bias, c_off=l * H)
            hip.gemm(hr, H, 1, W, 1, 2 * H, hidden, 2 * H, B, H, H, beta=1.0, act=2, b_off=H, c_off=l * H)
        saved["finals"] = finals
        saved["hidden"] = hidden
        return saved["layers"][1]["out"], hidden, saved

    def _keys(self, S, prefix, enc2d, H):
        W = S[prefix + ".attn.weight"]
        K = self._empty(enc2d.shape[0], H, dev=enc2d.device)
        hip.gemm(enc2d, 2 * H, 1, W, 1, 4 * H, K, H, enc2d.shape[0], H, 2 * H, b_off=2 * H, act=3,
                 two_term=(hip.one(enc2d.device), hip.absmax(W)) if _ENC_TWO_TERM else None)
        return K

    def _staff_token(self, S, ids, lengths, len_stride, out, col0, maxlen, id_bstride, ids_are_i64, record=None):
        L = hip.lib()
        names = [f"decoder.staff_emb.{w}_{sfx}" for sfx in ("l0", "l0_reverse") for w in ("weight_ih", "weight_hh", "bias_ih", "bias_hh")]
        arr = (C.c_void_p * 8)(*[S[n].data_ptr() for n in names])
        R = out.shape[0]
        E, Sz = self.cfg["note_emb_size"], self.cfg["staff_emb_size"]
        hsave = torch.empty((R, 2, maxlen, Sz), dtype=torch.float32, device=out.device) if record is not None else None
        hip.check(L.a2s_staff_emb_fwd(hip.stream(), hip._p(S["decoder.note_emb.weight"]), arr, hip._p(ids) if ids_are_i64 else None,
                                      None if ids_are_i64 else hip._p(ids), id_bstride, hip._p(lengths), len_stride, hip._p(out), out.stride(0), col0, hip._p(hsave), R,
                                      maxlen, E, Sz), "a2s_staff_emb_fwd")
        if record is not None:
            record.append(dict(ids=ids, lengths=lengths, len_stride=len_stride, col0=col0, maxlen=maxlen, id_bstride=id_bstride,
                               i64=ids_are_i64, hsave=hsave))

    def _decode_staff(self, S, prefix, keys, enc, h0, max_steps, probs_bar, gt_bar, steps, tf_flags, training, drop_p, B, T, attn_ws=None, gemm_ws=None,
                      active=None, drop=None, flags_dev=None, persist=False, defer_launch=False):
        L = hip.lib()
        H, E, V = self.cfg["hidden_size"], self.cfg["note_emb_size"], VOCAB_SIZE
        H2, ldx = 2 * H, E + 2 * H
        dev = enc.device
        n = steps
        graph = gt_bar is None and not training and getattr(self, "greedy_graph", _GREEDY_GRAPH)
        grammar = self.kern_grammar if (gt_bar is None and not training) else None
        if grammar is not None:
            if grammar.vocab_size != V:
                raise hip.A2SError(f"Engine.kern_grammar is a table over {grammar.vocab_size} symbols, the decoder's vocabulary has {V}")
            persist = False
        align = bool(self.alignment) and not training
        if align:
            if active is not None or defer_launch:
                raise hip.A2SError("alignment decodes bar by bar: no fused bars, no pair loop")
            persist, graph = False, False
        if gt_bar is None and not training and self._beam_slots():
            if active is not None or defer_launch:
                raise hip.A2SError("beam search decodes bar by bar: no fused bars, no pair loop")
            ids_, lengths_, saved = self._decode_staff_beam(S, prefix, keys, enc, h0, max_steps, probs_bar, n, B, T, grammar, self._beam_slots())
            if align:
                gt_ids = ids_.long()
                n_forced = plan_note_steps(gt_ids.cpu(), max_steps)[0]
                scratch = torch.zeros((B, max_steps, V), dtype=torch.float32, device=dev)
                forced = self._decode_staff(S, prefix, keys, enc, h0, max_steps, scratch, gt_ids, n_forced, [1] * n_forced, False, 0.0, B, T,
                                            attn_ws=attn_ws, gemm_ws=gemm_ws)[2]
                saved["align"], saved["align_forced"] = forced["align"], forced
            return ids_, lengths_, saved
        t_base = torch.zeros(1, dtype=torch.int32, device=dev) if graph else None
        h = self._empty(n + 1, B, H2, dev=dev)
        h[0].copy_(h0)
        x = self._empty(n + 1, B, ldx, dev=dev)
        q = self._empty(n, B, H, dev=dev)
        o = self._empty(n, B, 2 * H2, dev=dev)
        gates = self._empty(n, B, 4 * H2, dev=dev) if training else None
        attw = self._empty(n, B, T, dev=dev) if training else None
        gh, gi = self._empty(B, 3 * H2, dev=dev), self._empty(B, 3 * H2, dev=dev)
        logits = self._empty(B, V, dev=dev)
        ids = torch.zeros((B, max_steps), dtype=torch.int32, device=dev) if grammar is None else torch.full((B, max_steps), PAD, dtype=torch.int32, device=dev)
        eos_seen = torch.zeros(B, dtype=torch.int32, device=dev)
        lengths = torch.full((B,), max_steps, dtype=torch.long, device=dev)
        n_done = torch.zeros(1, dtype=torch.int32, device=dev)
        steps_exec = torch.zeros(1, dtype=torch.int32, device=dev)
        if drop is None and training and drop_p > 0:
            drop = (torch.rand((n + 1, B, E), device=dev) >= drop_p).to(torch.uint8)
        hip.check(L.a2s_embed_rows(hip.stream(), hip._p(S[prefix + ".embedding.weight"]), None, None, 0, SOS, hip._p(x), ldx, 0, B, E, hip._p(drop),
                                   1.0 / (1.0 - drop_p) if drop is not None else 1.0), "a2s_embed_rows")
        flags = (C.c_uint8 * max(n, 1))(*([int(f) for f in tf_flags] if tf_flags is not None else [0] * n))
        a = hip.NoteDecArgs()
        for name, t in (("attn_w", S[prefix + ".attn.attn.weight"]), ("attn_b", S[prefix + ".attn.attn.bias"]),
                        ("attn_v", S[prefix + ".attn.v.weight"]), ("w_ih", S[prefix + ".gru.weight_ih_l0"]),
                        ("w_hh", S[prefix + ".gru.weight_hh_l0"]), ("b_ih", S[prefix + ".gru.bias_ih_l0"]),
                        ("b_hh", S[prefix + ".gru.bias_hh_l0"]), ("out_w", S[prefix + ".out.weight"]), ("out_b", S[prefix + ".out.bias"]),
                        ("emb", S[prefix + ".embedding.weight"]), ("keys", keys), ("enc", enc), ("h", h), ("x", x), ("q", q),
                        ("gates", gates), ("attw", attw), ("o", o), ("gh", gh), ("gi", gi), ("logits", logits),
                        ("argmax_out", ids), ("eos_seen", eos_seen), ("lengths", lengths), ("n_done", n_done), ("steps_exec", steps_exec), ("drop", drop), ("attn_ws", attn_ws), ("gemm_ws", gemm_ws), ("t_base", t_base),
                        ("clip_order", active and active["order"]), ("clip_rank", active and active["rank"]),
                        ("row_until", active and active["until"])):
            setattr(a, name, t.data_ptr() if t is not None else None)
        a.gemm_ws_bytes = gemm_ws.numel() * 4 if gemm_ws is not None else 0
        step_ws = hip.step_workspace(H, E, dev)
        a.step_ws, a.step_ws_floats = step_ws.data_ptr(), step_ws.numel()
        a.n_active = C.cast(active["n_active"], C.c_void_p).value if active else None
        a.n_clips = active["n_clips"] if active else 0
        a.m_active = C.cast(active["m_active"], C.c_void_p).value if (active and active.get("m_active") is not None) else None
        if active and active.get("row_list") is not None:
            a.row_list, a.n_rows_active = active["row_list"].data_ptr(), C.cast(active["n_rows_active"], C.c_void_p).value
        else:
            a.row_list, a.n_rows_active = None, None
        a.probs, a.probs_bstride = probs_bar.data_ptr(), probs_bar.stride(0)
        if gt_bar is not None:
            a.gt, a.gt_bstride = gt_bar.data_ptr(), gt_bar.stride(0)
        else:
            a.gt, a.gt_bstride = None, 0
        a.tf_flags = C.cast(flags, C.c_void_p).value
        a.inv_keep = 1.0 / (1.0 - drop_p) if drop is not None else 1.0
        a.am_bstride = max_steps
        a.R, a.T, a.H, a.E, a.V, a.steps, a.poll, a.eos_id = B, T, H, E, V, n, (self.poll if gt_bar is None else 0), EOS
        a.use_graph = 1 if graph else 0
        persist_ws = None
        a.tf_flags_dev, a.persist_ws, a.persist_ws_bytes = None, None, 0
        if persist and n > 0 and (gt_bar is not None or not training) and (tf_flags is None or flags_dev is not None):
            nb_ws = L.a2s_note_decoder_persist_ws_bytes(active["n_clips"] if active else B, B, n)
            if nb_ws:
                persist_ws = torch.empty(nb_ws, dtype=torch.uint8, device=dev)
                a.persist_ws, a.persist_ws_bytes = persist_ws.data_ptr(), nb_ws
                a.tf_flags_dev = flags_dev.data_ptr() if flags_dev is not None else None
        def finish(launched):
            executed = n if gt_bar is not None else int(steps_exec.item())
            if gt_bar is None and a.persist_ws:
                hip.check_persist_abort(dev, raise_error=True)
            saved = dict(h=h, x=x, q=q, o=o, gates=gates, attw=attw, drop=drop, steps=executed, launched=launched, ids=ids, flags=list(flags),
                         gt_bar=gt_bar, prefix=prefix, max_steps=max_steps, drop_p=drop_p, attn_ws=attn_ws, gemm_ws=gemm_ws, active=active, flags_dev=flags_dev,
                         step_ws=step_ws, persist_ws=persist_ws, logits=logits, gh=gh, gi=gi, eos_seen=eos_seen, n_done=n_done)
            return ids, lengths, saved
        if defer_launch:
            return a, finish
        done = C.c_int(0)
        if align:
            g, at = hip.align_buffers(B, max_steps, T, dev)
            row_state = None
            if grammar is not None:
                row_state = torch.full((B,), grammar.start, dtype=torch.int32, device=dev)
                g.next_state, g.n_states, g.row_state = grammar.device_table(dev).data_ptr(), grammar.n_states, row_state.data_ptr()
            hip.check(L.a2s_note_decoder_fwd_align(hip.stream(), C.byref(a), C.byref(g), C.byref(done)), "a2s_note_decoder_fwd_align")
            ids_, lengths_, saved = finish(done.value)
            saved["align"] = at
            if row_state is not None:
                saved["row_state"] = row_state
            return ids_, lengths_, saved
        if grammar is not None:
            row_state = torch.full((B,), grammar.start, dtype=torch.int32, device=dev)
            hip.check(L.a2s_note_decoder_fwd_grammar(hip.stream(), C.byref(a), hip._p(grammar.device_table(dev)), grammar.n_states, hip._p(row_state),
                                                     C.byref(done)), "a2s_note_decoder_fwd_grammar")
            ids_, lengths_, saved = finish(done.value)
            saved["row_state"] = row_state
            return ids_, lengths_, saved
        hip.check(L.a2s_note_decoder_fwd(hip.stream(), C.byref(a), C.byref(done)), "a2s_note_decoder_fwd")
        return finish(done.value)

    def _beam_slots(self):
        K = self.beam_size
        if not isinstance(K, int) or isinstance(K, bool) or not 1 <= K <= 4:
            raise ValueError(f"Engine.beam_size must be an integer in 1 .. 4 (got {K!r})")
        return K if (K >= 2 or _BEAM_FORCE) else 0

    def _decode_staff_beam(self, S, prefix, keys, enc, h0, max_steps, probs_bar, n, B, T, grammar, K):
        L = hip.lib()
        H, E, V = self.cfg["hidden_size"], self.cfg["note_emb_size"], VOCAB_SIZE
        H2, ldx = 2 * H, E + 2 * H
        dev = enc.device
        R = K * B
        h = self._empty(2, R, H2, dev=dev)
        h[0].view(K, B, H2).copy_(h0.unsqueeze(0).expand(K, B, H2))
        x = self._empty(2, R, ldx, dev=dev)
# ... 415 lines not shown
```

piano_a2s_amd/engine_bwd.py:

```python
import ctypes as C
import os
import threading

import torch

from . import hip
from .spec import SOS, VOCAB_SIZE


def _os_env(name, default):
    return os.environ.get(name, default)


def _ptr(t, off=0):
    return C.c_void_p(t.data_ptr() + 4 * off)


_COLSUM_WS = {}


def _colsum(x, ld, out, rows, ncol, x_off=0, out_off=0, beta=1.0):
    ws = None
    if rows >= 2048:
        key = (x.device, torch.cuda.current_stream().cuda_stream, threading.get_ident())
# ... 274 lines not shown
        deferred_streams = _deferred_streams(dev, gidx) if use_deferred_g else None
        deferred_done = []
        seg_dh0 = {}

        def segment_decoders_bwd(si_seg):
            seg = gs["segments"][si_seg]
            bar0, nb = seg["bars"][0], len(seg["bars"])
            calls = []
            for si, (name, prefix, dout, out_t) in enumerate((("up", "decoder.upper_decoder", dup_g, up_out_g), ("lo", "decoder.lower_decoder", dlo_g, lo_out_g))):
                if bar_major:
                    maxs = out_t.shape[2]
                    dpr, pr = dout[bar0:bar0 + nb].view(nb * Bg, maxs, -1), out_t[bar0:bar0 + nb].view(nb * Bg, maxs, -1)
                else:
                    dpr, pr = dout[:, bar0], out_t[:, bar0]
                calls.append((eng, S, Gg, seg["staff"][name][2], keys_g[prefix], enc_g, dpr, pr, dK_g[prefix], dEnc_staff_g[si], Bg, T,
                              deferred_streams[si] if use_deferred_g else None, enc_amax_g, self.late if self.late_wgrads else None))
            if concurrent_g and seg.get("pair") is not None and L.a2s_debug_get(b"attn_pair"):
                (res,), events = fork_on_streams(dev, [streams[1]], [lambda: _note_decoder_bwd_pair(calls, streams, seg["pair"])])(wait=False)
                seg_dh0[si_seg] = ([r[0] for r in res], events)
                deferred_done.extend(r[1] for r in res if r[1] is not None)
            elif concurrent_g:
                res, events = fork_on_streams(dev, streams, [lambda args=args: _note_decoder_bwd(*args) for args in calls])(wait=False)
                seg_dh0[si_seg] = ([r[0] for r in res], events)
                deferred_done.extend(r[1] for r in res if r[1] is not None)
            else:
                seg_dh0[si_seg] = ([_note_decoder_bwd(*args)[0] for args in calls], [])

        for si_seg in reversed(range(len(gs["segments"]))):
            segment_decoders_bwd(si_seg)

        bar_attn = []
        d_hid_carry = None
        d_token_next = None
        for bar in reversed(range(bars)):
            b = gs["bars"][bar]
            if d_token_next is not None:
                for rec in b["tok_rec"]:
                    _staff_token_bwd(eng, S, Gg, rec, d_token_next)
                ts_ids, key_ids, i64, stride = b["next_ids"]
                for table, ids_, col, width in (("decoder.time_sig_emb.weight", ts_ids, 4 * Sz, te), ("decoder.key_emb.weight", key_ids, 4 * Sz + te, ke)):
                    hip.check(L.a2s_embed_scatter_add(hip.stream(), hip._p(Gg[table]), hip._p(ids_) if i64 else None, None if i64 else hip._p(ids_), stride, 0,
                                                      hip._p(d_token_next), tokw, col, Bg, width, None, 1.0), "scatter ts/key")
            d_headin = torch.zeros((Bg, 4 * H), dtype=torch.float32, device=dev)
            for hname, dout, out_t, nc in (("time_sig_out", dts_g, ts_out_g, cfg["num_time_sig"]), ("key_out", dkey_g, key_out_g, cfg["num_keys"])):
                t1, t2, lg, _ = b["heads"][hname]
                dlg = torch.empty((Bg, nc), dtype=torch.float32, device=dev)
                hip.check(L.a2s_log_softmax_bwd_rows(hip.stream(), _ptr(dout, bar * nc), _ptr(out_t, bar * nc), bars * nc, 1, hip._p(dlg), Bg, nc, Bg, 0),
                          "lsm bwd head")
                p = f"decoder.{hname}"
                dt2 = torch.empty_like(t2)
                _linear_bwd(t2, S[p + ".4.weight"], dlg, Gg, p + ".4.weight", p + ".4.bias", dx=dt2)
                hip.check(L.a2s_ew_act_bwd(hip.stream(), hip._p(dt2), hip._p(t2), hip._p(dt2), dt2.numel(), 1), "relu bwd")
                dt1 = torch.empty_like(t1)
                _linear_bwd(t1, S[p + ".2.weight"], dt2, Gg, p + ".2.weight", p + ".2.bias", dx=dt1)
                hip.check(L.a2s_ew_act_bwd(hip.stream(), hip._p(dt1), hip._p(t1), hip._p(dt1), dt1.numel(), 1), "relu bwd")
                _linear_bwd(b["headin"], S[p + ".0.weight"], dt1, Gg, p + ".0.weight", p + ".0.bias", dx=d_headin, dx_beta=1.0)
            d_hnew = torch.zeros((Bg, H2), dtype=torch.float32, device=dev)
            si_seg, j = b["seg"]
            dh0s, events = seg_dh0[si_seg]
            for ev in events:
                torch.cuda.current_stream().wait_event(ev)
            for dh0 in dh0s:
                d_hnew.add_(dh0[j * Bg:(j + 1) * Bg])
            d_hnew.add_(d_headin[:, :H2])
            if d_hid_carry is not None:
                d_hnew.add_(d_hid_carry)
            ldxb = tokw + H2
            dgi, dgh = torch.empty((Bg, 3 * H2), device=dev), torch.empty((Bg, 3 * H2), device=dev)
            dhp = torch.empty((Bg, H2), device=dev)
            hip.check(L.a2s_gru_gates_bwd(hip.stream(), hip._p(d_hnew), H2, None, 0, hip._p(b["gates"]), hip._p(b["hprev"]), H2, hip._p(dgi), 3 * H2, hip._p(dgh),
                                          3 * H2, None, 0, hip._p(dhp), H2, Bg, H2), "gates bwd bar")
            d_xbar = torch.empty((Bg, ldxb), device=dev)
            _linear_bwd(b["xbar"], S["decoder.gru.weight_ih_l0"], dgi, Gg, "decoder.gru.weight_ih_l0", "decoder.gru.bias_ih_l0", dx=d_xbar)
            _linear_bwd(b["hprev"], S["decoder.gru.weight_hh_l0"], dgh, Gg, "decoder.gru.weight_hh_l0", "decoder.gru.bias_hh_l0", dx=dhp, dx_beta=1.0)
            dq, ds = torch.empty((Bg, H), device=dev), torch.empty((1, Bg, T), device=dev)
            dctx = torch.empty((1, Bg, H2), device=dev)
            from .engine import bar_attn_workspace
            bar_ws = bar_attn_workspace(dev, gidx, Bg, T, H)
            if bar_ws is not None:
                ctx_c, dctx_c = b["xbar"][:, tokw:].contiguous(), d_xbar[:, tokw:].contiguous()
                hip.check(L.a2s_attn_step_bwd(hip.stream(), hip._p(keys_g["decoder"]), hip._p(enc_g), hip._p(b["qb"]), H, hip._p(S["decoder.attn.v.weight"]),
                                              hip._p(b["attw"]), hip._p(ctx_c), H2, hip._p(dctx_c), H2, _ptr(d_headin, H2), 4 * H, hip._p(dctx), H2, hip._p(dq), H,
                                              hip._p(ds), Bg, T, H, hip._p(bar_ws)), "attn bwd bar")
            else:
                hip.check(L.a2s_attn_step_bwd(hip.stream(), hip._p(keys_g["decoder"]), hip._p(enc_g), hip._p(b["qb"]), H, hip._p(S["decoder.attn.v.weight"]),
                                              hip._p(b["attw"]), _ptr(b["xbar"], tokw), ldxb, _ptr(d_xbar, tokw), ldxb, _ptr(d_headin, H2), 4 * H, hip._p(dctx), H2,
                                              hip._p(dq), H, hip._p(ds), Bg, T, H, None), "attn bwd bar")
            Wa = S["decoder.attn.attn.weight"]
            hip.gemm(dq, H, 1, Wa, 4 * H, 1, dhp, H2, Bg, H2, H, beta=1.0)
            hip.gemm(dq, 1, H, b["hprev"], H2, 1, Gg["decoder.attn.attn.weight"], 4 * H, H, H2, Bg, beta=1.0)
            _colsum(dq, H, Gg["decoder.attn.attn.bias"], Bg, H)
            bar_attn.append((b["qb"].view(1, Bg, H), ds, b["attw"].view(1, Bg, T), dctx))
            d_hid_carry = dhp
            d_token = d_xbar[:, :tokw].contiguous()
            if b["keep"] is not None:
                d_token = d_token * b["keep"] / 0.9
            d_token_next = d_token
        qs, dss, aws, dcs = [torch.cat(t, 0) for t in zip(*bar_attn)]
        _attn_deferred(eng, S, Gg, "decoder.attn", keys_g["decoder"], enc_g, qs, dss, aws, dcs, dK_g["decoder"], dEnc_g, Bg, T, H, len(bar_attn))
        d_sos = d_token_next.clone()
        d_sos[:, :2 * Sz] += d_sos[:, 2 * Sz:4 * Sz]
        _staff_token_bwd(eng, S, Gg, gs["sos_rec"][0], d_sos)
        for table, cid, col, width in (("decoder.time_sig_emb.weight", cfg["num_time_sig"], 4 * Sz, te), ("decoder.key_emb.weight", cfg["num_keys"], 4 * Sz + te, ke)):
            hip.check(L.a2s_embed_scatter_add(hip.stream(), hip._p(Gg[table]), None, None, 0, cid, hip._p(d_token_next), tokw, col, Bg, width, None, 1.0),
                      "scatter sos ts/key")
        d_hidden[b0:b1].copy_(d_hid_carry)
        for ev in deferred_done:
            torch.cuda.current_stream().wait_event(ev)
        return None


    def finish(self, grad_ready=None):
        eng, S, G, dev = self.eng, self.S, self.G, self.dev
        B, T, F = self.B, self.T, self.F
        names, offs, total, flat = self.names, self.offs, self.total, self.flat
        dEnc, dK = self.dEnc, self.dK
        sv = eng.saved
        assert sv["training"], "backward needs a forward run with training=True (batch statistics / saved activations)"
        L = hip.lib()
        H = eng.cfg["hidden_size"]
        H2 = 2 * H
        enc = sv["enc_out"]
        G["__staff_emb_ptrs__"] = self.group_ptrs[0]
        late_join = None
        if self.late:
            dec_lo = next(off for k, off in zip(names, offs) if k.startswith("decoder."))
            assert all(k.startswith("decoder.") for k, off in zip(names, offs) if off >= dec_lo), "the decoder's parameters must be the tail of the flat layout"
            wg = _weight_grad_stream(dev)
            wg.wait_stream(torch.cuda.current_stream())
            with torch.cuda.stream(wg):
                for fn, ev, tensors in self.late:
                    wg.wait_event(ev)
                    for t in tensors:
                        if t is not None:
                            t.record_stream(wg)
                    fn()
            late_join = dec_lo
            self.late = []
        else:
            for gf in self.group_flat[1:]:
                flat.add_(gf)
        d_hid_carry = self.d_hidden
        if self.concurrent:
            dEnc.add_(self.dEnc_staff[0]).add_(self.dEnc_staff[1])
        enc2d = enc.view(B * T, H2)
        enc_amax = hip.absmax(enc) if self.two_term else None
        for p, dKp in dK.items():
            Wn = p + ".attn.attn.weight"
            dk_amax = hip.absmax(dKp) if self.two_term else None
            if not hip.tallk_wgrad(dKp, 0, H, enc2d, 0, H2, G[Wn], H2, 4 * H, B * T, H, H2, dk_amax, enc_amax):
                sk = L.a2s_gemm_pick_splitk(H, H2, B * T, 1)
                hip.gemm(dKp, 1, H, enc2d, H2, 1, G[Wn], 4 * H, H, H2, B * T, beta=1.0, splitk=sk, c_off=H2,
                         two_term=(dk_amax, enc_amax) if self.two_term else None)
            hip.gemm(dKp, H, 1, S[Wn], 4 * H, 1, dEnc, H2, B * T, H2, H, beta=1.0, b_off=H2,
                     two_term=(dk_amax, hip.absmax(S[Wn])) if self.two_term else None)
        if late_join is not None:
            wg = _weight_grad_stream(dev)
            wg.wait_stream(torch.cuda.current_stream())
            with torch.cuda.stream(wg):
                for gf in self.group_flat[1:]:
                    flat[late_join:].add_(gf[late_join:])
                if Backward.check_fold:
                    for gi, gf in enumerate(self.group_flat[1:], 1):
                        assert not bool(gf[:late_join].any()), f"clip group {gi}: non-decoder gradients in the group buffer would be lost by the late fold"
        defer = True
        d_conv = _encoder_bwd(eng, S, G, sv["enc"], dEnc, d_hid_carry, B, T, wait_weight_grads=not defer)
        n_conv = next(off for k, off in zip(names, offs) if not k.startswith("convstack."))
        if grad_ready is not None:
            if defer:
                with torch.cuda.stream(_weight_grad_stream(dev)):
                    grad_ready(self.flat_full, n_conv, total + 1)
            else:
                grad_ready(self.flat_full, n_conv, total + 1)
        if getattr(eng, "conv_unperm", None) is not None:
            d_conv = d_conv.reshape(B, T, -1).index_select(0, eng.conv_unperm)
        _convstack_bwd(eng, S, G, sv["conv"], d_conv, B, T, F)
        if defer:
            torch.cuda.current_stream().wait_stream(_weight_grad_stream(dev))
        if grad_ready is not None:
            grad_ready(flat, 0, n_conv)
        G[None] = flat
        G["__loss_gate__"] = self.flat_full[total:]
        eng._keep_alive = self.keep_alive
        return G




def backward(eng, S, grad_outputs, grad_ready=None, loss_total=None):
    from .engine import group_views, run_clip_groups
    sv = eng.saved
    assert sv["training"], "backward needs a forward run with training=True (batch statistics / saved activations)"
    dev = sv["enc_out"].device
    clip_groups = sv.get("clip_groups") or [(0, sv["shape"][0])]
    ctx = Backward(eng, S, sv["shape"], dev, clip_groups, sv.get("concurrent"), sv.get("bar_major"))
    dts, dkey, dup, dlo = [g.contiguous() for g in grad_outputs]

    def group(gidx):
        b0, b1 = clip_groups[gidx]
        if ctx.bar_major:
            dup_g, dlo_g = group_views(dup, clip_groups, gidx), group_views(dlo, clip_groups, gidx)
        else:
            dup_g, dlo_g = dup[b0:b1], dlo[b0:b1]
        ctx.decoder_group(gidx, sv["groups"][gidx], dts[b0:b1], dkey[b0:b1], dup_g, dlo_g)

    run_clip_groups(dev, [lambda gi=gi: group(gi) for gi in range(len(clip_groups))])
    if loss_total is not None:
        ctx.flat_full[ctx.total:].copy_(loss_total.reshape(1))
    return ctx.finish(grad_ready)


_WG_STREAMS = {}
_DEFERRED_STREAMS = {}


def _deferred_streams(dev, group=0):
    idx = torch.device(dev).index if torch.device(dev).index is not None else torch.cuda.current_device()
    key = (idx, group)
    if key not in _DEFERRED_STREAMS:
        _DEFERRED_STREAMS[key] = (torch.cuda.Stream(device=idx), torch.cuda.Stream(device=idx))
    return _DEFERRED_STREAMS[key]



def _weight_grad_stream(dev):
    from .engine import group_stream
    return group_stream(dev, 1)


def _encoder_bwd(eng, S, G, es, dEnc, d_hidden, B, T, wait_weight_grads=True):
    L = hip.lib()
    H = eng.cfg["hidden_size"]
    dev = dEnc.device
    W = S["encoder.fc.weight"]
    dpre = torch.empty_like(d_hidden)
    hip.check(L.a2s_ew_act_bwd(hip.stream(), hip._p(d_hidden), hip._p(es["hidden"]), hip._p(dpre), dpre.numel(), 2), "tanh bwd")
    dhn = []
    for l in (0, 1):
        for half, hfin in enumerate((es["finals"][2 * l], es["finals"][2 * l + 1])):
            d = torch.empty((B, H), device=dev)
            hip.gemm(dpre, 2 * H, 1, W, 2 * H, 1, d, H, B, H, H, a_off=l * H, b_off=half * H)
            hip.gemm(dpre, 1, 2 * H, hfin, H, 1, G["encoder.fc.weight"], 2 * H, H, H, B, beta=1.0, a_off=l * H, c_off=half * H)
            dhn.append(d)
        _colsum(dpre, 2 * H, G["encoder.fc.bias"], B, H, x_off=l * H)
    gws = [hip.gemm_workspace(B, dev), hip.gemm_workspace(B, dev)]
    two_term = True
    in_amax = hip.absmax(es["layers"][0]["in"]) if two_term else None
    dout = dEnc
    for layer in (1, 0):
        ls = es["layers"][layer]
        inp = ls["in"]
        I = inp.shape[1]
        out = ls["out"]
        dX = torch.empty((B * T, I), device=dev)
        from .engine import encoder_streams, fork_on_streams
        streams = encoder_streams(dev, B)

        def direction(d, sfx):
            dgi = torch.empty((B, T, 3 * H), device=dev)
            dghs = torch.empty((B, T, 3 * H), device=dev)
            dgh_first, dhbuf, dgh_tmp = torch.empty((B, 3 * H), device=dev), torch.empty((2, B, H), device=dev), torch.empty((B, 3 * H), device=dev)
            ranges, valid = torch.empty(2, device=dev), C.c_int(0)
            if two_term and L.a2s_debug_get(b"tallk_wgrad") > 0:
                hip.check(L.a2s_gru_seq_bwd_ranged(hip.stream(), _ptr(dout, d * H), T * 2 * H, 2 * H, _ptr(out, d * H), T * 2 * H, 2 * H, hip._p(ls["dirs"][d]["gates"]),
                                                   hip._p(S[f"encoder.gru.weight_hh_{sfx}"]), hip._p(dhn[2 * layer + d]), hip._p(dgi), hip._p(dghs), hip._p(dgh_first),
                                                   hip._p(dhbuf), hip._p(dgh_tmp), B, T, H, d, hip._p(gws[d]), gws[d].numel() * 4, hip._p(ranges), C.byref(valid)),
                          "a2s_gru_seq_bwd_ranged")
            else:
                hip.check(L.a2s_gru_seq_bwd(hip.stream(), _ptr(dout, d * H), T * 2 * H, 2 * H, _ptr(out, d * H), T * 2 * H, 2 * H, hip._p(ls["dirs"][d]["gates"]),
                                            hip._p(S[f"encoder.gru.weight_hh_{sfx}"]), hip._p(dhn[2 * layer + d]), hip._p(dgi), hip._p(dghs), hip._p(dgh_first),
                                            hip._p(dhbuf), hip._p(dgh_tmp), B, T, H, d, hip._p(gws[d]), gws[d].numel() * 4), "a2s_gru_seq_bwd")
            return (dgi, dghs, dgh_first, dhbuf, dgh_tmp, ranges if valid.value else None)

        res = fork_on_streams(dev, streams, [lambda d=d, sfx=sfx: direction(d, sfx) for d, sfx in enumerate((f"l{layer}", f"l{layer}_reverse"))])()
        dgi_amax = []
        for d, sfx in enumerate((f"l{layer}", f"l{layer}_reverse")):
            dgi2 = res[d][0].view(B * T, 3 * H)
            Wih = S[f"encoder.gru.weight_ih_{sfx}"]
            ranges = res[d][5]
            tt = (ranges[0:1] if ranges is not None else hip.absmax(dgi2), hip.absmax(Wih)) if two_term else None
            dgi_amax.append(tt[0] if tt else None)
            if L.a2s_debug_get(b"gemm_bf16x3") > 0:
                hip.gemm(dgi2, 3 * H, 1, Wih.t().contiguous(), 1, 3 * H, dX, I, B * T, I, 3 * H, beta=0.0 if d == 0 else 1.0, two_term=tt)
            else:
                hip.gemm(dgi2, 3 * H, 1, Wih, I, 1, dX, I, B * T, I, 3 * H, beta=0.0 if d == 0 else 1.0, two_term=tt)
        wg = _weight_grad_stream(dev)
        ev = torch.cuda.Event()
        ev.record()
        wg.wait_event(ev)
        for d, sfx in enumerate((f"l{layer}", f"l{layer}_reverse")):
            dgi, dghs, dgh_first, ranges = res[d][0], res[d][1], res[d][2], res[d][5]
            for t in (dgi, dghs, dgh_first, dgi_amax[d], in_amax, ranges):
                if t is not None:
                    t.record_stream(wg)
            with torch.cuda.stream(wg):
                dgi2, dghs2 = dgi.view(B * T, 3 * H), dghs.view(B * T, 3 * H)
                x_bound = ((in_amax if layer == 0 else hip.one(dev)) if two_term else None)
                if not hip.tallk_wgrad(inp, 0, I, dgi2, 0, 3 * H, G[f"encoder.gru.weight_ih_{sfx}"], 0, I, B * T, I, 3 * H, x_bound, dgi_amax[d],
                                       transposed=True, bias=G[f"encoder.gru.bias_ih_{sfx}"]):
                    _linear_bwd(inp, S[f"encoder.gru.weight_ih_{sfx}"], dgi2, G, f"encoder.gru.weight_ih_{sfx}", f"encoder.gru.bias_ih_{sfx}",
                                dy_amax=dgi_amax[d], x_bound=x_bound)
                dghs_amax = (ranges[1:2] if ranges is not None else hip.absmax(dghs2)) if two_term else None
                if not hip.tallk_wgrad(out, d * H, 2 * H, dghs2, 0, 3 * H, G[f"encoder.gru.weight_hh_{sfx}"], 0, H, B * T, H, 3 * H,
                                       hip.one(dev) if two_term else None, dghs_amax, transposed=True, bias=G[f"encoder.gru.bias_hh_{sfx}"]):
                    sk = L.a2s_gemm_pick_splitk(3 * H, H, B * T, 1)
                    hip.gemm(dghs2, 1, 3 * H, out, 2 * H, 1, G[f"encoder.gru.weight_hh_{sfx}"], H, 3 * H, H, B * T, beta=1.0, splitk=sk, b_off=d * H,
                             two_term=(dghs_amax, hip.one(dev)) if two_term else None)
                    _colsum(dghs2, 3 * H, G[f"encoder.gru.bias_hh_{sfx}"], B * T, 3 * H)
                _colsum(dgh_first, 3 * H, G[f"encoder.gru.bias_hh_{sfx}"], B, 3 * H)
        dout = dX.view(B, T, I)
    if wait_weight_grads:
        torch.cuda.current_stream().wait_stream(_weight_grad_stream(dev))
    return dout


_FUSE_BN_APPLY = False
_FUSE_BN_APPLY_L1 = True
_DGRAD_BNSTATS = True
_SYNC_FUSED = True
_LIN_WGRAD_AT = "before"
_FUSE_BN_ROWS = os.environ.get("A2S_FUSE_BN_ROWS", "1") != "0"


def _linear_dgrad_generic(L, dev, rows, F, Cf, dz, Wout, da, y4, bn4, dz_amax, w_amax):
    nblk = L.a2s_gemm_bnstats_blocks(rows, F)
    part = torch.empty((nblk, 40, 2), dtype=torch.float32, device=dev)
    if L.a2s_debug_get(b"gemm_bf16x3") > 0:
        Wt = Wout.t().contiguous()
        wb, s_bk, s_bn = Wt, 1, Cf
    else:
        wb, s_bk, s_bn = Wout, 40 * F, 1
    hip.check(L.a2s_gemm_f32_bnstats_scaled(hip.stream(), rows, 40 * F, Cf, hip._p(dz), Cf, 1, hip._p(wb), s_bk, s_bn, hip._p(da), 40 * F, hip._p(y4), hip._p(bn4[0]),
                                            hip._p(bn4[1]), hip._p(bn4[2]), hip._p(bn4[3]), F, hip._p(part), hip._p(dz_amax), hip._p(w_amax)),
              "a2s_gemm_f32_bnstats_scaled")
    return part, nblk


def _convstack_bwd(eng, S, G, cs, d_out, B, T, F):
    L = hip.lib()
    dev = d_out.device
    Cf = eng.cfg["conv_feature_size"]
    rows = B * T

    def bn_bwd(g, x, bn, name, mask, n_rows, C_, F_, stats_only=False, partial=None, amax=None):
        mean, invstd, scale, shift = bn
        if partial is not None and eng.sync_bn and stats_only:
            import torch.distributed as dist
            local = torch.empty(2 * C_, dtype=torch.float32, device=dev)
            hip.check(L.a2s_bn_bwd_sums_from_partial(hip.stream(), hip._p(partial[0]), partial[1], C_, hip._p(local)), "a2s_bn_bwd_sums_from_partial")
            glob = local.clone()
            dist.all_reduce(glob)
            c12 = torch.empty(2 * C_, dtype=torch.float32, device=dev)
            hip.check(L.a2s_bn_bwd_c12_from_sums(hip.stream(), hip._p(local), hip._p(glob), eng.bn_counts[name], hip._p(G[name + ".weight"]), hip._p(G[name + ".bias"]),
                                                 hip._p(c12), C_), "a2s_bn_bwd_c12_from_sums")
            return c12
        if partial is not None and not eng.sync_bn:
            c12 = torch.empty(2 * C_, dtype=torch.float32, device=dev)
            hip.check(L.a2s_bn_bwd_from_partial_amax(hip.stream(), hip._p(g), hip._p(x), hip._p(mean), hip._p(invstd), hip._p(scale), hip._p(shift),
                                                     hip._p(G[name + ".weight"]), hip._p(G[name + ".bias"]), None if stats_only else hip._p(g), hip._p(partial[0]),
                                                     partial[1], hip._p(c12), n_rows, C_, F_, hip._p(amax)), "a2s_bn_bwd_from_partial")
            return c12 if stats_only else g
        part = torch.empty(L.a2s_bn_bwd_partial_floats(n_rows, C_, F_), dtype=torch.float32, device=dev)
        c12 = torch.empty(2 * C_, dtype=torch.float32, device=dev)
        if eng.sync_bn:
            import torch.distributed as dist
            local = torch.empty(2 * C_, dtype=torch.float32, device=dev)
            hip.check(L.a2s_bn_bwd_stats(hip.stream(), hip._p(g), hip._p(x), hip._p(mean), hip._p(invstd), hip._p(scale), hip._p(shift), hip._p(mask), 1.0 / 0.8,
                                         hip._p(part), hip._p(local), n_rows, C_, F_), "a2s_bn_bwd_stats")
            glob = local.clone()
            dist.all_reduce(glob)
            hip.check(L.a2s_bn_bwd_apply(hip.stream(), hip._p(g), hip._p(x), hip._p(mean), hip._p(invstd), hip._p(scale), hip._p(shift), hip._p(mask), 1.0 / 0.8,
                                         hip._p(local), hip._p(glob), eng.bn_counts[name], hip._p(G[name + ".weight"]), hip._p(G[name + ".bias"]), hip._p(g),
                                         hip._p(c12), n_rows, C_, F_), "a2s_bn_bwd_apply")
            return g
        hip.check(L.a2s_bn_bwd_amax(hip.stream(), hip._p(g), hip._p(x), hip._p(mean), hip._p(invstd), hip._p(scale), hip._p(shift), hip._p(mask), 1.0 / 0.8,
                                    hip._p(G[name + ".weight"]), hip._p(G[name + ".bias"]), None if stats_only else hip._p(g), hip._p(part), hip._p(c12), n_rows, C_, F_,
                                    hip._p(amax)), "a2s_bn_bwd")
        return c12 if stats_only else g

    g = d_out.reshape(rows, Cf).contiguous()
    dz_amax = torch.zeros(1, dtype=torch.float32, device=dev)
    dz = bn_bwd(g, cs["z"], cs["out_bn"], "convstack.out_bn", cs["drop"], rows, Cf, 1, amax=dz_amax)
    if eng.sync_bn:
        hip.absmax(dz, dz_amax)
    w_amax = cs.get("w_out_amax")
    a4 = cs["a4"]
    g_partial = None
    g_amax = None
    Wout = S["convstack.out.weight"]
    if a4 is None:
        y4 = cs["y"][3].view(rows, 40 * F)
        da = torch.empty_like(y4)
        bn4 = cs["bn"][3]
        def lin_wgrad():
            if not hip.linear_wgrad(dz, y4, (bn4[2], bn4[3], F), dz_amax, cs["abound"][3], G["convstack.out.weight"]):
                _linear_bwd(y4, Wout, dz, G, "convstack.out.weight", None, x_affine=(bn4[2], bn4[3], F), dy_amax=dz_amax, x_bound=cs["abound"][3])
        lin_at = _LIN_WGRAD_AT
        lin_overlap = lin_at != "before"

        def lin_wgrad_side():
            wg_stream = _weight_grad_stream(dev)
            ev = torch.cuda.Event()
            ev.record()
            wg_stream.wait_event(ev)
            with torch.cuda.stream(wg_stream):
                lin_wgrad()
        if lin_at == "beside":
            lin_wgrad_side()
        elif lin_at == "before":
            lin_wgrad()
        if _DGRAD_BNSTATS and (not eng.sync_bn or _SYNC_FUSED) and F >= 128 and F % 4 == 0 and rows > 64:
            if w_amax is None:
                w_amax = hip.absmax(Wout)
            if hip.LINEAR_KERNELS and L.a2s_linear_dgrad_eligible(rows, 40 * F, Cf, F):
                nblk = L.a2s_linear_dgrad_blocks(rows)
                part = torch.empty((nblk, 40, 2), dtype=torch.float32, device=dev)
                Wt = Wout.t().contiguous()
                nb = L.a2s_linear_dgrad_ws_bytes(40 * F, Cf)
                lws = torch.empty(nb // 4, dtype=torch.float32, device=dev)
                g_amax = torch.zeros(1, dtype=torch.float32, device=dev)
                hip.check(L.a2s_linear_dgrad_bnstats(hip.stream(), rows, 40 * F, Cf, hip._p(dz), Cf, hip._p(Wt), hip._p(da), 40 * F, hip._p(y4), hip._p(bn4[0]),
                                                     hip._p(bn4[1]), hip._p(bn4[2]), hip._p(bn4[3]), F, hip._p(part), hip._p(dz_amax), hip._p(w_amax), hip._p(lws), nb,
                                                     hip._p(g_amax)), "a2s_linear_dgrad_bnstats")
                g_partial = (part, nblk)
            else:
                g_partial = _linear_dgrad_generic(L, dev, rows, F, Cf, dz, Wout, da, y4, bn4, dz_amax, w_amax)
        else:
            hip.gemm(dz, Cf, 1, Wout, 40 * F, 1, da, 40 * F, rows, 40 * F, Cf)
    else:
        da = torch.empty_like(a4)
        _linear_bwd(a4, Wout, dz, G, "convstack.out.weight", None, dx=da)
    chans = [(1, 20), (20, 20), (20, 40), (40, 40)]
    g = da.view(B, T, 40, F)
    for i in (4, 3, 2, 1):
        ci, co = chans[i - 1]
# ... 53 lines not shown
```

piano_a2s_amd/hip.py:

```python
import ctypes as C
import os
import threading

import torch

from .abi import PROTOTYPES, STRUCTS, A2SError
from .build import LIB

LIB = os.environ.get("A2S_LIB", LIB)

NoteDecArgs, NoteDecBwdArgs, BeamArgs, AlignArgs = (STRUCTS[n] for n in ("a2s_note_dec_args", "a2s_note_dec_bwd_args", "a2s_beam_args", "a2s_align_args"))
_lib = None


def lib():
    global _lib
    if _lib is None:
        if not os.path.exists(LIB):
            raise A2SError(f"HIP extension not built: {LIB} is missing (run `python __graft_entry__.py build`). "
                           "There is no CPU fallback for the transcription hot path.")
        arith = os.environ.get("A2S_ARITH", "f16x2")
        if arith not in ("f16x2", "bf16x3", "f32"):
            raise A2SError(f"A2S_ARITH={arith!r}: expected f16x2, bf16x3 or f32")
        L = C.CDLL(LIB)
# ... 241 lines not shown


def gemm(A, sAm, sAk, B, sBk, sBn, Cout, ldc, M, N, K, alpha=1.0, beta=0.0, bias=None, act=0,
         batch=1, bsA=0, bsB=0, bsC=0, splitk=1, a_off=0, b_off=0, c_off=0, a_affine=None, b_affine=None, two_term=None):
    L = lib()
    ws, ws_bytes = None, 0
    if splitk > 1:
        ws_bytes = L.a2s_gemm_workspace_bytes(M, N, batch, splitk)
        ws = torch.empty(ws_bytes // 4, dtype=torch.float32, device=Cout.device)
    pa = C.c_void_p(A.data_ptr() + 4 * a_off)
    pb = C.c_void_p(B.data_ptr() + 4 * b_off)
    pc = C.c_void_p(Cout.data_ptr() + 4 * c_off)
    if a_affine is None and b_affine is None and two_term is None:
        check(L.a2s_gemm_f32(stream(), M, N, K, alpha, pa, sAm, sAk, pb, sBk, sBn, beta, pc, ldc, _p(bias), act, batch, bsA, bsB, bsC, splitk, _p(ws), ws_bytes),
              "a2s_gemm_f32")
        return
    asc, ash, ap = a_affine if a_affine is not None else (None, None, 0)
    bsc, bsh, bp = b_affine if b_affine is not None else (None, None, 0)
    if two_term is not None:
        check(L.a2s_gemm_f32_affine_scaled(stream(), M, N, K, alpha, pa, sAm, sAk, pb, sBk, sBn, beta, pc, ldc, _p(bias), act, batch, bsA, bsB, bsC, splitk, _p(ws),
                                           ws_bytes, _p(asc), _p(ash), ap, _p(bsc), _p(bsh), bp, _p(two_term[0]), _p(two_term[1])), "a2s_gemm_f32_affine_scaled")
        return
    check(L.a2s_gemm_f32_affine(stream(), M, N, K, alpha, pa, sAm, sAk, pb, sBk, sBn, beta, pc, ldc, _p(bias), act, batch, bsA, bsB, bsC, splitk, _p(ws), ws_bytes,
                                _p(asc), _p(ash), ap, _p(bsc), _p(bsh), bp), "a2s_gemm_f32_affine")


_ONES = {}


def one(device):
    key = torch.device(device).index
    if key not in _ONES:
        _ONES[key] = torch.ones(1, dtype=torch.float32, device=device)
    return _ONES[key]


def absmax(x, out=None):
    if out is None:
        out = torch.empty(1, dtype=torch.float32, device=x.device)
    check(lib().a2s_absmax(stream(), _p(x), x.numel(), _p(out)), "a2s_absmax")
    return out


def linear(x2d, weight, bias=None, act=0, out=None, beta=0.0, x_affine=None, two_term=None):
    M, K = x2d.shape
    N = weight.shape[0]
    if out is None:
        out = torch.empty((M, N), dtype=torch.float32, device=x2d.device)
    gemm(x2d, x2d.stride(0), x2d.stride(1), weight, weight.stride(1), weight.stride(0), out, out.stride(0), M, N, K,
         bias=bias, act=act, beta=beta, a_affine=x_affine, two_term=two_term)
    return out


def conv3x3_forward(x, w, y, scale, shift, partial, cws, in_absmax=None, out_absmax=None):
    B, T, Cin, F = x.shape
    check(lib().a2s_conv3x3_ranged(stream(), _p(x), _p(w), _p(y), _p(scale), _p(shift), _p(in_absmax), _p(partial), _p(out_absmax),
                                   B, T, F, Cin, y.shape[2], _p(cws)), "a2s_conv3x3_ranged")


def conv3x3_dgrad_for_test(dy, w, yl):
    L = lib()
    B, T, Cout, F = dy.shape
    Cin = w.shape[1]
    dev = dy.device
    dx = torch.full((B, T, Cin, F), float("nan"), device=dev)
    amax = absmax(dy)
    part = torch.zeros(L.a2s_conv3x3_stat_blocks(B, T, F, Cout), Cin, 2, device=dev)
    cws = conv_workspace(Cout, dev)
    zeros, ones = torch.zeros(Cin, device=dev), torch.ones(Cin, device=dev)
    check(L.a2s_conv3x3_dgrad_bnstats_scaled(stream(), _p(dy), _p(w), _p(dx), _p(yl), _p(zeros), _p(ones), _p(ones), _p(zeros), _p(part),
                                             B, T, F, Cout, Cin, _p(cws), _p(amax)), "a2s_conv3x3_dgrad_bnstats_scaled")
    torch.cuda.synchronize()
    return dx


def act_bound(scale, shift, x_absmax):
    out = torch.empty(1, dtype=torch.float32, device=scale.device)
    check(lib().a2s_act_bound(stream(), _p(scale), _p(shift), _p(x_absmax), scale.numel(), _p(out)), "a2s_act_bound")
    return out


def conv3x3_wgrad(dy, x, scale, shift, dW, ws, dy_absmax, act_absmax):
    B, T, Cout, F = dy.shape
    Cin = x.shape[2]
    check(lib().a2s_conv3x3_wgrad_ranged(stream(), _p(dy), _p(x), _p(scale), _p(shift), _p(dW), _p(ws), ws.numel() * 4, B, T, F, Cin, Cout, _p(dy_absmax),
                                         _p(act_absmax)), "a2s_conv3x3_wgrad_ranged")


def conv3x3_wgrad_for_test(dy, x, scale, shift):
    L = lib()
    B, T, Cout, F = dy.shape
    Cin = x.shape[2]
    dev = dy.device
    dW = torch.zeros(Cout, Cin, 3, 3, device=dev)
    ws = torch.empty(L.a2s_conv3x3_wgrad_workspace_bytes(Cin, Cout) // 4, device=dev)
    bound = act_bound(scale, shift, x.abs().amax(dim=(0, 1, 3)).contiguous())
    conv3x3_wgrad(dy, x, scale, shift, dW, ws, absmax(dy), bound)
    torch.cuda.synchronize()
    return dW


def linear_forward(x2d, weight, x_affine, x_bound, w_absmax, out=None):
    M, K = x2d.shape
    N = weight.shape[0]
    L = lib()
    period = x_affine[2]
    if (LINEAR_KERNELS and x2d.is_contiguous() and weight.is_contiguous() and x_bound is not None
            and L.a2s_linear_fwd_eligible(M, N, K, period)):
        if out is None:
            out = torch.empty((M, N), dtype=torch.float32, device=x2d.device)
        nb = L.a2s_linear_dgrad_ws_bytes(N, K)
        ws = torch.empty(nb // 4, dtype=torch.float32, device=x2d.device)
        check(L.a2s_linear_fwd(stream(), M, N, K, _p(x2d), K, _p(weight), _p(out), N, _p(x_affine[0]), _p(x_affine[1]), period, _p(x_bound), _p(w_absmax), _p(ws), nb),
              "a2s_linear_fwd")
        return out
    return linear(x2d, weight, out=out, x_affine=x_affine, two_term=(x_bound, w_absmax))


def linear_wgrad(dz, x2d, x_affine, dz_absmax, x_bound, G):
    M, K = x2d.shape
    N = dz.shape[1]
    L = lib()
    if (not LINEAR_KERNELS or not (x2d.is_contiguous() and dz.is_contiguous() and G.is_contiguous()) or dz_absmax is None
            or x_bound is None or not L.a2s_linear_wgrad_eligible(M, N, K, x_affine[2])):
        return False
    nb = L.a2s_linear_wgrad_ws_bytes(M, K)
    ws = torch.empty(nb // 4, dtype=torch.float32, device=x2d.device)
    check(L.a2s_linear_wgrad(stream(), M, N, K, _p(dz), N, _p(x2d), K, _p(G), K, _p(x_affine[0]), _p(x_affine[1]), x_affine[2], _p(dz_absmax), _p(x_bound), _p(ws), nb),
          "a2s_linear_wgrad")
    return True


_TALLK_WS = {}


def tallk_wgrad(P, p_off, ldp, A, a_off, lda, G, g_off, ldg, M, Np, K, p_absmax, a_absmax, transposed=False, bias=None):
    L = lib()
    if not hasattr(L, "a2s_tallk_wgrad_eligible"):
        return False
    pp, pa, pg = P.data_ptr() + 4 * p_off, A.data_ptr() + 4 * a_off, G.data_ptr() + 4 * g_off
    if (p_absmax is None or a_absmax is None or (pp | pa | pg | (bias.data_ptr() if bias is not None else 0)) % 16
            or not L.a2s_tallk_wgrad_eligible(M, Np, K, ldp, lda, ldg, int(transposed))):
        return False
    nb = L.a2s_tallk_wgrad_ws_bytes(M, Np, K)
    key = (A.device, torch.cuda.current_stream().cuda_stream, threading.get_ident())
    ws = _TALLK_WS.get(key)
    if ws is None or ws.numel() * 4 < nb:
        ws = _TALLK_WS[key] = torch.empty((nb + 3) // 4, dtype=torch.float32, device=A.device)
    check(L.a2s_tallk_wgrad(stream(), M, Np, K, C.c_void_p(pp), ldp, C.c_void_p(pa), lda, C.c_void_p(pg), ldg, int(transposed), _p(bias), _p(p_absmax), _p(a_absmax),
                            _p(ws), ws.numel() * 4), "a2s_tallk_wgrad")
    return True


def linear_forward_for_test(x, w, aff):
    period = aff[2]
    xmax = x.view(x.shape[0], -1, period).abs().amax(dim=(0, 2)).contiguous()
    return linear_forward(x, w, aff, act_bound(aff[0], aff[1], xmax), absmax(w))
```

Baseline: 639.4.

## Add persistent tall-M f16x2 GEMM path for encoder projections and grads

```diff
diff --git a/include/a2s.h b/include/a2s.h
--- a/include/a2s.h
+++ b/include/a2s.h
@@ -45,6 +45,10 @@
                     const float* p_absmax, const float* a_absmax, float* workspace, size_t workspace_bytes);
 size_t a2s_tallk_wgrad_ws_bytes(int M, int Np, int K);
 int a2s_tallk_wgrad_eligible(int M, int Np, int K, long ldp, long lda, long ldg, int transposed);
+int a2s_tallm_gemm(void* stream, int M, int N, int K, const float* A, long lda, const float* B, long sBk, long sBn, float* C, long ldc, const float* bias,
+                   int beta, int act, const float* a_absmax, const float* b_absmax, float* workspace, size_t workspace_bytes);
+size_t a2s_tallm_gemm_ws_bytes(int N, int K);
+int a2s_tallm_gemm_eligible(int M, int N, int K, long lda, long sBk, long sBn, long ldc, int beta, int act);
 size_t a2s_linear_dgrad_ws_bytes(int N, int K);
 int a2s_linear_dgrad_blocks(int M);
 int a2s_linear_dgrad_eligible(int M, int N, int K, int period);
diff --git a/piano_a2s_amd/csrc/a2s_api.hip b/piano_a2s_amd/csrc/a2s_api.hip
--- a/piano_a2s_amd/csrc/a2s_api.hip
+++ b/piano_a2s_amd/csrc/a2s_api.hip
@@ -65,6 +65,14 @@
 size_t a2s_tallk_wgrad_ws_bytes(int M, int Np, int K) { return a2s_tallk_wgrad_ws_bytes_impl(M, Np, K); }
 int a2s_tallk_wgrad_eligible(int M, int Np, int K, long ldp, long lda, long ldg, int transposed) {
     return a2s_tallk_wgrad_ok(M, Np, K, ldp, lda, ldg, transposed, nullptr, nullptr, nullptr, nullptr) ? 1 : 0;
+}
+int a2s_tallm_gemm(void* stream, int M, int N, int K, const float* A, long lda, const float* B, long sBk, long sBn, float* C, long ldc, const float* bias,
+                   int beta, int act, const float* a_absmax, const float* b_absmax, float* workspace, size_t workspace_bytes) {
+    return a2s_tallm_gemm_impl(ST, M, N, K, A, lda, B, sBk, sBn, C, ldc, bias, beta, act, a_absmax, b_absmax, workspace, workspace_bytes);
+}
+size_t a2s_tallm_gemm_ws_bytes(int N, int K) { return a2s_tallm_gemm_ws_bytes_impl(N, K); }
+int a2s_tallm_gemm_eligible(int M, int N, int K, long lda, long sBk, long sBn, long ldc, int beta, int act) {
+    return a2s_tallm_gemm_ok(M, N, K, lda, sBk, sBn, ldc, beta, act, nullptr, nullptr, nullptr) ? 1 : 0;
 }
 int a2s_linear_fwd_eligible(int M, int N, int K, int period) { return a2s_linear_fwd_ok(M, N, K, 4, 4, period, nullptr, nullptr, nullptr) ? 1 : 0; }
 int a2s_linear_dgrad_blocks(int M) { return a2s_linear_dgrad_blocks_impl(M); }
@@ -88,6 +96,8 @@
     if (!strcmp(key, "attn_deferred_fast")) { a2s_attn_deferred_fast = value ? 1 : 0; return A2S_OK; }
     if (!strcmp(key, "tallk_wgrad")) { a2s_tallk_wgrad_on = value ? 1 : 0; return A2S_OK; }
     if (!strcmp(key, "tallk_wgrad_max_splits")) { a2s_tallk_wgrad_max_splits = value > 0 ? value : 0; return A2S_OK; }
+    if (!strcmp(key, "tallm_gemm")) { a2s_tallm_gemm_on = value ? 1 : 0; return A2S_OK; }
+    if (!strcmp(key, "tallm_gemm_max_wgs")) { a2s_tallm_gemm_max_wgs = value > 0 ? value : 0; return A2S_OK; }
     if (!strcmp(key, "gemm_tile")) { a2s_gemm_debug_tile_impl(value); return A2S_OK; }
     snprintf(a2s_err_msg, sizeof(a2s_err_msg), "a2s_debug_set: unknown key %s", key);
     return A2S_ERR_ARG;
@@ -110,6 +120,9 @@
     if (!strcmp(key, "tallk_wgrad")) return a2s_tallk_wgrad_on;
     if (!strcmp(key, "tallk_wgrad_max_splits")) return a2s_tallk_wgrad_max_splits;
     if (!strcmp(key, "tallk_wgrad_launches")) return (int)a2s_tallk_wgrad_launches();
+    if (!strcmp(key, "tallm_gemm")) return a2s_tallm_gemm_on;
+    if (!strcmp(key, "tallm_gemm_max_wgs")) return a2s_tallm_gemm_max_wgs;
+    if (!strcmp(key, "tallm_gemm_launches")) return (int)a2s_tallm_gemm_launches();
     if (!strcmp(key, "attn_dk_ahead_launches")) return (int)a2s_attn_dk_ahead_launches();
     if (!strcmp(key, "attn_denc_launches")) return (int)a2s_attn_denc_launches();
     if (!strcmp(key, "dec_mid_launches")) return a2s_dec_mid_launches();
diff --git a/piano_a2s_amd/csrc/a2s_internal.h b/piano_a2s_amd/csrc/a2s_internal.h
--- a/piano_a2s_amd/csrc/a2s_internal.h
+++ b/piano_a2s_amd/csrc/a2s_internal.h
@@ -39,6 +39,13 @@
 bool a2s_linear_wgrad_ok(int M, int N, int K, long ldz, long lda, long ldg, int period, const void* dz, const void* A, const void* G);
 int a2s_linear_wgrad_impl(hipStream_t st, int M, int N, int K, const float* dz, long ldz, const float* A, long lda, float* G, long ldg, const float* a_scale,
     const float* a_shift, int period, const float* dz_absmax, const float* a_absmax, float* ws, size_t ws_bytes);
+extern int a2s_tallm_gemm_on;
+extern int a2s_tallm_gemm_max_wgs;
+long a2s_tallm_gemm_launches(void);
+size_t a2s_tallm_gemm_ws_bytes_impl(int N, int K);
+bool a2s_tallm_gemm_ok(int M, int N, int K, long lda, long sBk, long sBn, long ldc, int beta, int act, const void* A, const void* B, const void* C);
+int a2s_tallm_gemm_impl(hipStream_t st, int M, int N, int K, const float* A, long lda, const float* B, long sBk, long sBn, float* C, long ldc,
+    const float* bias, int beta, int act, const float* a_absmax, const float* b_absmax, float* ws, size_t ws_bytes);
 extern int a2s_tallk_wgrad_on;
 extern int a2s_tallk_wgrad_max_splits;
 long a2s_tallk_wgrad_launches(void);
diff --git a/piano_a2s_amd/csrc/a2s_linear.hip b/piano_a2s_amd/csrc/a2s_linear.hip
--- a/piano_a2s_amd/csrc/a2s_linear.hip
+++ b/piano_a2s_amd/csrc/a2s_linear.hip
@@ -20,15 +20,21 @@
     float* c_absmax_out;
 };
 
-__global__ __launch_bounds__(256) void lin_pack_planes_k(const float* __restrict__ W, long ld, int N, int K, const float* __restrict__ absmax,
+__global__ __launch_bounds__(256) void lin_pack_planes_k(const float* __restrict__ W, long ld, long sk, int N, int K, const float* __restrict__ absmax,
                                                          unsigned char* __restrict__ out) {
     const long id = (long)blockIdx.x * 256 + threadIdx.x;
     const int kgroups = K >> 3, nks = K >> 5;
-    const int n = (int)(id / kgroups), kg = (int)(id % kgroups);
-    if (n >= N) return;
+    const int n = sk == 1 ? (int)(id / kgroups) : (int)(id % N), kg = sk == 1 ? (int)(id % kgroups) : (int)(id / N);
+    if (n >= N || kg >= kgroups) return;
     const float ps = ldexpf(1.f, pow2_scale_exp(*absmax, 12));
-    const f32x4 v0 = *reinterpret_cast<const f32x4*>(W + (long)n * ld + kg * 8);
-    const f32x4 v1 = *reinterpret_cast<const f32x4*>(W + (long)n * ld + kg * 8 + 4);
+    f32x4 v0, v1;
+    if (sk == 1) {
+        v0 = *reinterpret_cast<const f32x4*>(W + (long)n * ld + kg * 8);
+        v1 = *reinterpret_cast<const f32x4*>(W + (long)n * ld + kg * 8 + 4);
+    } else {
+#pragma unroll
+        for (int i = 0; i < 4; ++i) { v0[i] = W[(long)n * ld + (long)(kg * 8 + i) * sk]; v1[i] = W[(long)n * ld + (long)(kg * 8 + 4 + i) * sk]; }
+    }
     float x[8];
 #pragma unroll
     for (int i = 0; i < 4; ++i) { x[i] = __builtin_amdgcn_fmed3f(v0[i] * ps, -65000.f, 65000.f); x[4 + i] = __builtin_amdgcn_fmed3f(v1[i] * ps, -65000.f, 65000.f); }
@@ -195,7 +201,7 @@
     hipError_t e = hipMemsetAsync(partial, 0, sizeof(float) * 2 * (size_t)nblk * channels, st);
     if (e != hipSuccess) A2S_FAIL(A2S_ERR_HIP, "linear_dgrad_bnstats memset: %s", hipGetErrorString(e));
     unsigned char* planes = reinterpret_cast<unsigned char*>(ws);
-    hipLaunchKernelGGL(lin_pack_planes_k, dim3((unsigned)(((long)N * (K / 8) + 255) / 256)), dim3(256), 0, st, Wt, (long)K, N, K, b_absmax, planes);
+    hipLaunchKernelGGL(lin_pack_planes_k, dim3((unsigned)(((long)N * (K / 8) + 255) / 256)), dim3(256), 0, st, Wt, (long)K, 1L, N, K, b_absmax, planes);
     A2S_CHECK_LAUNCH("lin_pack_planes_k");
     LinDgradArgs a{A, lda, planes, C, ldc, ep_y, mean, invstd, scale, shift, partial, a_absmax, b_absmax, M, N, period, channels, c_absmax_out};
     hipLaunchKernelGGL(lin_dgrad_bnstats, dim3((M + LIN_BM - 1) / LIN_BM), dim3(LIN_NTH), 0, st, a);
@@ -214,42 +220,57 @@
     const float* a_scale; const float* a_shift;
     const float* a_absmax; const float* b_absmax;
     int M, K, period;
+    const float* bias; int beta, act;
 };
 
+template <bool TALLM>
 __global__ __launch_bounds__(LIN_NTH) void lin_fwd_roles(LinFwdArgs a) {
     __shared__ __attribute__((aligned(16))) unsigned char lds[LF_NS * LF_STAGE];
     const int tid = threadIdx.x, lane = tid & 63, lr = lane & 15, lk = lane >> 4;
     const int wave = __builtin_amdgcn_readfirstlane(tid >> 6);
-    const int m0 = blockIdx.x * LIN_BM;
     const int ka = a.a_absmax ? pow2_scale_exp(*a.a_absmax, 12) : 0, kb = pow2_scale_exp(*a.b_absmax, 12);
     const float psa = ldexpf(1.f, ka), unscale = ldexpf(1.f, -(ka + kb));
     const int nks = a.K >> 5, nblk = a.K >> 6, kpc = a.period >> 5;
     const bool affine = a.a_scale != nullptr;
+    const int nrb = (a.M + LIN_BM - 1) / LIN_BM;
+    const int nit = TALLM ? (nrb - (int)blockIdx.x + (int)gridDim.x - 1) / (int)gridDim.x : 1;
+    const int total = nit * nblk;
     if (wave >= 4) {
         const int st_ = tid - 256;
         const int sk = (st_ & 15) * 4;
         const bool second = sk >= 32;
+        const bool stream_a = !TALLM || gridDim.y == 1;
         f32x4 ar[2][8];
-        auto issue_a = [&](int blk, f32x4 (&r)[8]) {
+        auto issue_a = [&](int g, f32x4 (&r)[8]) {
+            const int it = TALLM ? g / nblk : 0, blk = g - it * nblk;
+            const int m0 = ((int)blockIdx.x + it * (int)gridDim.x) * LIN_BM;
 #pragma unroll
             for (int i = 0; i < 8; ++i) {
                 const int row = (st_ + 256 * i) >> 4;
                 r[i] = (f32x4){0.f, 0.f, 0.f, 0.f};
-                if (m0 + row < a.M && blk < nblk) r[i] = __builtin_nontemporal_load(reinterpret_cast<const f32x4*>(a.A + (long)(m0 + row) * a.lda + (long)blk * 64 + sk));
+                if (m0 + row < a.M && g < total) {
+                    const f32x4* src = reinterpret_cast<const f32x4*>(a.A + (long)(m0 + row) * a.lda + (long)blk * 64 + sk);
+                    r[i] = stream_a ? __builtin_nontemporal_load(src) : *src;
+                }
             }
         };
-        auto commit_a = [&](int blk, const f32x4 (&r)[8]) {
-            if (blk >= nblk) return;
+        auto commit_a = [&](int g, const f32x4 (&r)[8]) {
+            if (g >= total) return;
+            const int blk = TALLM ? g % nblk : g;
             const int c0 = (2 * blk) / kpc, c1 = (2 * blk + 1) / kpc;
             const float sc = affine ? (second ? a.a_scale[c1] : a.a_scale[c0]) * psa : psa, sh = affine ? (second ? a.a_shift[c1] : a.a_shift[c0]) * psa : 0.f;
             const float floor_ = affine ? 0.f : -INFINITY;
-            unsigned char* st = lds + (blk % LF_NS) * LF_STAGE;
+            const bool negate = TALLM && ((blk >> 2) & 1);
+            unsigned char* st = lds + (g % LF_NS) * LF_STAGE;
 #pragma unroll
             for (int i = 0; i < 8; ++i) {
                 const int row = (st_ + 256 * i) >> 4;
                 float x[4];
 #pragma unroll
-                for (int j = 0; j < 4; ++j) x[j] = __builtin_amdgcn_fmed3f(fmaxf(fmaf(r[i][j], sc, sh), floor_), -65000.f, 65000.f);
+                for (int j = 0; j < 4; ++j) {
+                    x[j] = __builtin_amdgcn_fmed3f(fmaxf(fmaf(r[i][j], sc, sh), floor_), -65000.f, 65000.f);
+                    if (TALLM) x[j] = negate ? -x[j] : x[j];
+                }
                 uint2 hi, lo;
                 split2_pair_f16(x[0], x[1], hi.x, lo.x);
                 split2_pair_f16(x[2], x[3], hi.y, lo.y);
@@ -261,30 +282,30 @@
         commit_a(0, ar[0]);
         issue_a(1, ar[1]); issue_a(2, ar[0]);
 #pragma unroll 1
-        for (int b0 = 0; b0 < nblk; b0 += 2) {
+        for (int b0 = 0; b0 < total; b0 += 2) {
             __syncthreads();
             commit_a(b0 + 1, ar[1]); issue_a(b0 + 3, ar[1]);
-            if (b0 + 1 < nblk) {
+            if (b0 + 1 < total) {
                 __syncthreads();
                 commit_a(b0 + 2, ar[0]); issue_a(b0 + 4, ar[0]);
             }
         }
         return;
     }
+    const int nt0 = (TALLM ? (int)blockIdx.y * 16 : 0) + wave * 4;
     lu32x4 bf[2][4][2];
     auto load_b = [&](int ks, lu32x4 (&dst)[4][2]) {
-        if (ks >= nks) return;
+        if (ks >= nks) {
+            if (!TALLM) return;
+            ks -= nks;
+        }
 #pragma unroll
         for (int nt = 0; nt < 4; ++nt)
 #pragma unroll
             for (int sp = 0; sp < 2; ++sp)
-                dst[nt][sp] = *reinterpret_cast<const lu32x4*>(a.planes + (((long)(wave * 4 + nt) * nks + ks) * 2 + sp) * 1024 + (unsigned)lane * 16u);
+                dst[nt][sp] = *reinterpret_cast<const lu32x4*>(a.planes + (((long)(nt0 + nt) * nks + ks) * 2 + sp) * 1024 + (unsigned)lane * 16u);
     };
     f32x4 acc[8][4];
-#pragma unroll
-    for (int mt = 0; mt < 8; ++mt)
-#pragma unroll
-        for (int nt = 0; nt < 4; ++nt) acc[mt][nt] = (f32x4){0.f, 0.f, 0.f, 0.f};
     load_b(0, bf[0]);
     auto load_af = [&](const unsigned char* st, int h, int qt, lu32x4 (&af)[2][2]) {
 #pragma unroll
@@ -301,42 +322,91 @@
         LR_PRODUCT(1, 0) LR_PRODUCT(0, 1) LR_PRODUCT(0, 0)
 #undef LR_PRODUCT
     };
+    auto flip = [&]() {
+#pragma unroll
+        for (int mt = 0; mt < 8; ++mt)
+#pragma unroll
+            for (int nt = 0; nt < 4; ++nt)
+#pragma unroll
+                for (int r = 0; r < 4; ++r) acc[mt][nt][r] = -acc[mt][nt][r];
+    };
+    int stage = 0;
 #pragma unroll 1
-    for (int blk = 0; blk < nblk; ++blk) {
-        __syncthreads();
-        const unsigned char* st = lds + (blk % LF_NS) * LF_STAGE;
-        lu32x4 fa[2][2], fb[2][2];
-        load_af(st, 0, 0, fa);
-        load_b(2 * blk + 1, bf[1]);
-        __builtin_amdgcn_sched_barrier(0);
-        load_af(st, 0, 1, fb); multiply(0, fa, bf[0]);
-        __builtin_amdgcn_sched_barrier(0);
-        load_af(st, 0, 2, fa); multiply(1, fb, bf[0]);
-        __builtin_amdgcn_sched_barrier(0);
-        load_af(st, 0, 3, fb); multiply(2, fa, bf[0]);
-        __builtin_amdgcn_sched_barrier(0);
-        load_af(st, 1, 0, fa); multiply(3, fb, bf[0]);
-        __builtin_amdgcn_sched_barrier(0);
-        load_b(2 * blk + 2, bf[0]);
-        load_af(st, 1, 1, fb); multiply(0, fa, bf[1]);
-        __builtin_amdgcn_sched_barrier(0);
-        load_af(st, 1, 2, fa); multiply(1, fb, bf[1]);
-        __builtin_amdgcn_sched_barrier(0);
-        load_af(st, 1, 3, fb); multiply(2, fa, bf[1]);
-        __builtin_amdgcn_sched_barrier(0);
-        multiply(3, fb, bf[1]);
-        __builtin_amdgcn_sched_barrier(0);
-    }
-#pragma unroll
-    for (int mt = 0; mt < 8; ++mt) {
-        const int m = m0 + mt * 16 + lr;
-        if (m >= a.M) continue;
-#pragma unroll
-        for (int nt = 0; nt < 4; ++nt) {
-            f32x4 v = acc[mt][nt];
-#pragma unroll
-            for (int r = 0; r < 4; ++r) v[r] *= unscale;
-            *reinterpret_cast<f32x4*>(a.C + (long)m * a.ldc + wave * 64 + nt * 16 + lk * 4) = v;
+    for (int it = 0; it < nit; ++it) {
+        const int m0 = ((int)blockIdx.x + it * (int)gridDim.x) * LIN_BM;
+#pragma unroll
+        for (int mt = 0; mt < 8; ++mt)
+#pragma unroll
+            for (int nt = 0; nt < 4; ++nt) acc[mt][nt] = (f32x4){0.f, 0.f, 0.f, 0.f};
+#pragma unroll 1
+        for (int blk = 0; blk < nblk; ++blk) {
+            if (TALLM && blk && !(blk & 3)) flip();
+            __syncthreads();
+            const unsigned char* st = lds + stage * LF_STAGE;
+            stage = stage + 1 == LF_NS ? 0 : stage + 1;
+            lu32x4 fa[2][2], fb[2][2];
+            load_af(st, 0, 0, fa);
+            load_b(2 * blk + 1, bf[1]);
+            __builtin_amdgcn_sched_barrier(0);
+            load_af(st, 0, 1, fb); multiply(0, fa, bf[0]);
+            __builtin_amdgcn_sched_barrier(0);
+            load_af(st, 0, 2, fa); multiply(1, fb, bf[0]);
+            __builtin_amdgcn_sched_barrier(0);
+            load_af(st, 0, 3, fb); multiply(2, fa, bf[0]);
+            __builtin_amdgcn_sched_barrier(0);
+            load_af(st, 1, 0, fa); multiply(3, fb, bf[0]);
+            __builtin_amdgcn_sched_barrier(0);
+            load_b(2 * blk + 2, bf[0]);
+            load_af(st, 1, 1, fb); multiply(0, fa, bf[1]);
+            __builtin_amdgcn_sched_barrier(0);
+            load_af(st, 1, 2, fa); multiply(1, fb, bf[1]);
+            __builtin_amdgcn_sched_barrier(0);
+            load_af(st, 1, 3, fb); multiply(2, fa, bf[1]);
+            __builtin_amdgcn_sched_barrier(0);
+            multiply(3, fb, bf[1]);
+            __builtin_amdgcn_sched_barrier(0);
+        }
+        if (TALLM && (((nblk - 1) >> 2) & 1)) flip();
+        if constexpr (!TALLM) {
+#pragma unroll
+            for (int mt = 0; mt < 8; ++mt) {
+                const int m = m0 + mt * 16 + lr;
+                if (m >= a.M) continue;
+#pragma unroll
+                for (int nt = 0; nt < 4; ++nt) {
+                    f32x4 v = acc[mt][nt];
+#pragma unroll
+                    for (int r = 0; r < 4; ++r) v[r] *= unscale;
+                    *reinterpret_cast<f32x4*>(a.C + (long)m * a.ldc + wave * 64 + nt * 16 + lk * 4) = v;
+                }
+            }
+        } else {
+#pragma unroll
+            for (int nt = 0; nt < 4; ++nt) {
+                const int n = (nt0 + nt) * 16 + lk * 4;
+                float bq[4] = {0.f, 0.f, 0.f, 0.f};
+                if (a.bias) {
+#pragma unroll
+                    for (int r = 0; r < 4; ++r) bq[r] = a.bias[n + r];
+                }
+#pragma unroll
+                for (int mt = 0; mt < 8; ++mt) {
+                    const int m = m0 + mt * 16 + lr;
+                    if (m >= a.M) continue;
+                    float* dst = a.C + (long)m * a.ldc + n;
+                    f32x4 v = acc[mt][nt];
+                    f32x4 old = {0.f, 0.f, 0.f, 0.f};
+                    if (a.beta) old = *reinterpret_cast<const f32x4*>(dst);
+#pragma unroll
+                    for (int r = 0; r < 4; ++r) {
+                        float x = v[r] * unscale + bq[r];
+                        if (a.beta) x += old[r];
+                        if (a.act == 3) x = exp2x_clamped(x);
+                        v[r] = x;
+                    }
+                    *reinterpret_cast<f32x4*>(dst) = v;
+                }
+            }
         }
     }
 }
@@ -353,11 +423,44 @@
                 "linear_fwd: needs N = 256, K %% 64 == 0, period %% 32 == 0 and 16-byte aligned rows");
     A2S_REQUIRE(((uintptr_t)ws % 16 == 0) && ws_bytes >= (size_t)N * K * 4, "linear_fwd: workspace too small (%zu bytes needed)", (size_t)N * K * 4);
     unsigned char* planes = reinterpret_cast<unsigned char*>(ws);
-    hipLaunchKernelGGL(lin_pack_planes_k, dim3((unsigned)(((long)N * (K / 8) + 255) / 256)), dim3(256), 0, st, W, (long)K, N, K, w_absmax, planes);
+    hipLaunchKernelGGL(lin_pack_planes_k, dim3((unsigned)(((long)N * (K / 8) + 255) / 256)), dim3(256), 0, st, W, (long)K, 1L, N, K, w_absmax, planes);
     A2S_CHECK_LAUNCH("lin_pack_planes_k");
-    LinFwdArgs a{A, lda, planes, C, ldc, a_scale, a_shift, a_absmax, w_absmax, M, K, a_scale ? period : K};
-    hipLaunchKernelGGL(lin_fwd_roles, dim3((M + LIN_BM - 1) / LIN_BM), dim3(LIN_NTH), 0, st, a);
+    LinFwdArgs a{A, lda, planes, C, ldc, a_scale, a_shift, a_absmax, w_absmax, M, K, a_scale ? period : K, nullptr, 0, 0};
+    hipLaunchKernelGGL(lin_fwd_roles<false>, dim3((M + LIN_BM - 1) / LIN_BM), dim3(LIN_NTH), 0, st, a);
     A2S_CHECK_LAUNCH("lin_fwd");
+    return A2S_OK;
+}
+
+int a2s_tallm_gemm_on = 1;
+int a2s_tallm_gemm_max_wgs = 0;
+static long long g_tallm_launches = 0;
+long a2s_tallm_gemm_launches(void) { return (long)__atomic_load_n(&g_tallm_launches, __ATOMIC_RELAXED); }
+
+bool a2s_tallm_gemm_ok(int M, int N, int K, long lda, long sBk, long sBn, long ldc, int beta, int act, const void* A, const void* B, const void* C) {
+    return a2s_tallm_gemm_on && M >= 1 && N >= 256 && N % 256 == 0 && N <= 4096 && (K == 256 || K == 512 || K == 768) && lda >= K && lda % 4 == 0 &&
+           ldc >= N && ldc % 4 == 0 && ((sBk == 1 && sBn >= K && sBn % 4 == 0) || (sBn == 1 && sBk >= N)) && (beta == 0 || beta == 1) &&
+           (act == 0 || act == 3) && (((uintptr_t)A | (uintptr_t)C) % 16 == 0) && (uintptr_t)B % (sBk == 1 ? 16 : 4) == 0;
+}
+size_t a2s_tallm_gemm_ws_bytes_impl(int N, int K) { return N > 0 && K > 0 ? (size_t)N * K * 4 : 0; }
+
+int a2s_tallm_gemm_impl(hipStream_t st, int M, int N, int K, const float* A, long lda, const float* B, long sBk, long sBn, float* C, long ldc,
+                        const float* bias, int beta, int act, const float* a_absmax, const float* b_absmax, float* ws, size_t ws_bytes) {
+    A2S_REQUIRE(A && B && C && b_absmax && ws, "tallm_gemm: null argument");
+    A2S_REQUIRE(a2s_tallm_gemm_ok(M, N, K, lda, sBk, sBn, ldc, beta, act, A, B, C),
+                "tallm_gemm: needs N %% 256 == 0, K in {256, 512, 768}, one unit stride of B, beta 0 or 1, act 0 or 3, 16-byte aligned rows (or the switch \"tallm_gemm\" is off)");
+    A2S_REQUIRE(((uintptr_t)ws % 16 == 0) && ws_bytes >= a2s_tallm_gemm_ws_bytes_impl(N, K), "tallm_gemm: workspace too small (%zu bytes needed)",
+                a2s_tallm_gemm_ws_bytes_impl(N, K));
+    unsigned char* planes = reinterpret_cast<unsigned char*>(ws);
+    hipLaunchKernelGGL(lin_pack_planes_k, dim3((unsigned)(((long)N * (K / 8) + 255) / 256)), dim3(256), 0, st, B, sBn, sBk, N, K, b_absmax, planes);
+    A2S_CHECK_LAUNCH("lin_pack_planes_k");
+    const int nrb = (M + LIN_BM - 1) / LIN_BM, ny = N / 256, cus = a2s_device_geometry().cus > 0 ? a2s_device_geometry().cus : 256;
+    int gx = cus / ny >= 8 ? (cus / ny) / 8 * 8 : 1;
+    if (a2s_tallm_gemm_max_wgs > 0 && gx > a2s_tallm_gemm_max_wgs) gx = a2s_tallm_gemm_max_wgs;
+    if (gx > nrb) gx = nrb;
+    LinFwdArgs a{A, lda, planes, C, ldc, nullptr, nullptr, a_absmax, b_absmax, M, K, K, bias, beta, act};
+    hipLaunchKernelGGL(lin_fwd_roles<true>, dim3(gx, ny), dim3(LIN_NTH), 0, st, a);
+    A2S_CHECK_LAUNCH("lin_fwd_roles<tallm>");
+    __atomic_fetch_add(&g_tallm_launches, 1LL, __ATOMIC_RELAXED);
     return A2S_OK;
 }
 
diff --git a/piano_a2s_amd/engine.py b/piano_a2s_amd/engine.py
--- a/piano_a2s_amd/engine.py
+++ b/piano_a2s_amd/engine.py
@@ -342,9 +342,17 @@
             out = self._empty(B, T, 2 * H, dev=dev)
             lsave = {"in": inp, "dirs": []}
             in_amax = (hip.absmax(inp) if layer == 0 else hip.one(dev)) if _ENC_TWO_TERM else None
-            gis = [hip.linear(inp, S[f"encoder.gru.weight_ih_{sfx}"], S[f"encoder.gru.bias_ih_{sfx}"],
-                              two_term=(in_amax, hip.absmax(S[f"encoder.gru.weight_ih_{sfx}"])) if _ENC_TWO_TERM else None)
-                   for sfx in (f"l{layer}", f"l{layer}_reverse")]
+            def project(sfx):
+                W, bias = S[f"encoder.gru.weight_ih_{sfx}"], S[f"encoder.gru.bias_ih_{sfx}"]
+                I = inp.shape[1]
+                if _ENC_TWO_TERM:
+                    w_amax = hip.absmax(W)
+                    gi = self._empty(B * T, 3 * H, dev=dev)
+                    if hip.tallm_gemm(inp, 0, I, W, 0, 1, I, gi, 0, 3 * H, B * T, 3 * H, I, in_amax, w_amax, bias=bias):
+                        return gi
+                    return hip.linear(inp, W, bias, out=gi, two_term=(in_amax, w_amax))
+                return hip.linear(inp, W, bias)
+            gis = [project(sfx) for sfx in (f"l{layer}", f"l{layer}_reverse")]
             def direction(d, sfx, gi):
                 hbuf = self._empty(2, B, H, dev=dev)
                 gh = self._empty(B, 3 * H, dev=dev)
@@ -376,8 +384,9 @@
     def _keys(self, S, prefix, enc2d, H):
         W = S[prefix + ".attn.weight"]
         K = self._empty(enc2d.shape[0], H, dev=enc2d.device)
-        hip.gemm(enc2d, 2 * H, 1, W, 1, 4 * H, K, H, enc2d.shape[0], H, 2 * H, b_off=2 * H, act=3,
-                 two_term=(hip.one(enc2d.device), hip.absmax(W)) if _ENC_TWO_TERM else None)
+        tt = (hip.one(enc2d.device), hip.absmax(W)) if _ENC_TWO_TERM else None
+        if tt is None or not hip.tallm_gemm(enc2d, 0, 2 * H, W, 2 * H, 1, 4 * H, K, 0, H, enc2d.shape[0], H, 2 * H, tt[0], tt[1], act=3):
+            hip.gemm(enc2d, 2 * H, 1, W, 1, 4 * H, K, H, enc2d.shape[0], H, 2 * H, b_off=2 * H, act=3, two_term=tt)
         return K
 
     def _staff_token(self, S, ids, lengths, len_stride, out, col0, maxlen, id_bstride, ids_are_i64, record=None):
diff --git a/piano_a2s_amd/engine_bwd.py b/piano_a2s_amd/engine_bwd.py
--- a/piano_a2s_amd/engine_bwd.py
+++ b/piano_a2s_amd/engine_bwd.py
@@ -450,8 +450,10 @@
                 sk = L.a2s_gemm_pick_splitk(H, H2, B * T, 1)
                 hip.gemm(dKp, 1, H, enc2d, H2, 1, G[Wn], 4 * H, H, H2, B * T, beta=1.0, splitk=sk, c_off=H2,
                          two_term=(dk_amax, enc_amax) if self.two_term else None)
-            hip.gemm(dKp, H, 1, S[Wn], 4 * H, 1, dEnc, H2, B * T, H2, H, beta=1.0, b_off=H2,
-                     two_term=(dk_amax, hip.absmax(S[Wn])) if self.two_term else None)
+            w_amax = hip.absmax(S[Wn]) if self.two_term else None
+            if not self.two_term or not hip.tallm_gemm(dKp, 0, H, S[Wn], H2, 4 * H, 1, dEnc, 0, H2, B * T, H2, H, dk_amax, w_amax, beta=1.0):
+                hip.gemm(dKp, H, 1, S[Wn], 4 * H, 1, dEnc, H2, B * T, H2, H, beta=1.0, b_off=H2,
+                         two_term=(dk_amax, w_amax) if self.two_term else None)
         if late_join is not None:
             wg = _weight_grad_stream(dev)
             wg.wait_stream(torch.cuda.current_stream())
@@ -578,7 +580,9 @@
             ranges = res[d][5]
             tt = (ranges[0:1] if ranges is not None else hip.absmax(dgi2), hip.absmax(Wih)) if two_term else None
             dgi_amax.append(tt[0] if tt else None)
-            if L.a2s_debug_get(b"gemm_bf16x3") > 0:
+            if tt and hip.tallm_gemm(dgi2, 0, 3 * H, Wih, 0, I, 1, dX, 0, I, B * T, I, 3 * H, tt[0], tt[1], beta=0.0 if d == 0 else 1.0):
+                pass
+            elif L.a2s_debug_get(b"gemm_bf16x3") > 0:
                 hip.gemm(dgi2, 3 * H, 1, Wih.t().contiguous(), 1, 3 * H, dX, I, B * T, I, 3 * H, beta=0.0 if d == 0 else 1.0, two_term=tt)
             else:
                 hip.gemm(dgi2, 3 * H, 1, Wih, I, 1, dX, I, B * T, I, 3 * H, beta=0.0 if d == 0 else 1.0, two_term=tt)
diff --git a/piano_a2s_amd/hip.py b/piano_a2s_amd/hip.py
--- a/piano_a2s_amd/hip.py
+++ b/piano_a2s_amd/hip.py
@@ -417,6 +417,27 @@
     return True
 
 
+_TALLM_WS = {}
+
+
+def tallm_gemm(A, a_off, lda, B, b_off, sBk, sBn, Cout, c_off, ldc, M, N, K, a_absmax, b_absmax, bias=None, beta=0.0, act=0):
+    L = lib()
+    if not hasattr(L, "a2s_tallm_gemm_eligible"):
+        return False
+    pa, pb, pc = A.data_ptr() + 4 * a_off, B.data_ptr() + 4 * b_off, Cout.data_ptr() + 4 * c_off
+    if (b_absmax is None or beta not in (0.0, 1.0) or (pa | pc) % 16 or pb % (16 if sBk == 1 else 4)
+            or not L.a2s_tallm_gemm_eligible(M, N, K, lda, sBk, sBn, ldc, int(beta), act)):
+        return False
+    nb = L.a2s_tallm_gemm_ws_bytes(N, K)
+    key = (A.device, torch.cuda.current_stream().cuda_stream, threading.get_ident())
+    ws = _TALLM_WS.get(key)
+    if ws is None or ws.numel() * 4 < nb:
+        ws = _TALLM_WS[key] = torch.empty((nb + 3) // 4, dtype=torch.float32, device=A.device)
+    check(L.a2s_tallm_gemm(stream(), M, N, K, C.c_void_p(pa), lda, C.c_void_p(pb), sBk, sBn, C.c_void_p(pc), ldc, _p(bias), int(beta), act, _p(a_absmax),
+                           _p(b_absmax), _p(ws), ws.numel() * 4), "a2s_tallm_gemm")
+    return True
+
+
 def linear_forward_for_test(x, w, aff):
     period = aff[2]
     xmax = x.view(x.shape[0], -1, period).abs().amax(dim=(0, 2)).contiguous()
```

After: 643.2 (median of 6 runs). About the same (+0.6%).
